# zgchen33/MCGaze

Measured on AMD Instinct MI355X. Metric: clips/sec (7x3x224x224), higher is better.
Workload: dtype f16x3; 1 GPU; full multiclue_gaze_r50 forward (R-50 + FPN + 4 decoder stages + gaze head), 64 clips/GPU x 7 frames x 3x224x224, 64 clips/step; clips_per_gpu=64, clip_length=7, global_clips=64, chunk_frames=0, parallelism=single GPU, trunk_streams=2

## Files before the change

### include/mcgaze_hip.h

```cpp
#ifndef MCGAZE_HIP_H
#define MCGAZE_HIP_H

#include <stddef.h>
#include <stdint.h>

#ifdef __cplusplus
extern "C" {
#endif

#define MCG_ABI_VERSION 18

enum { MCG_OK = 0, MCG_ERR_ARG = 1, MCG_ERR_HIP = 2, MCG_ERR_UNSUPPORTED = 3, MCG_ERR_WORKSPACE = 4 };
typedef enum { MCG_F32 = 0, MCG_BF16 = 1, MCG_F16X3 = 2, MCG_F16 = 3 } mcg_dtype;
#define MCG_ELEM_BYTES(dt) (((dt) == MCG_BF16 || (dt) == MCG_F16) ? 2 : 4)
typedef void* mcg_stream;

int mcg_abi_version(void);
const char* mcg_build_id(void);
const char* mcg_last_error(void);
int mcg_device_info(int* cu_count, size_t* hbm_bytes, char* arch, int arch_len);

int mcg_nchw_to_nhwc(mcg_stream s, mcg_dtype dt, const float* src, void* dst, int N, int C, int H, int W);
int mcg_nhwc_to_nchw(mcg_stream s, mcg_dtype dt, const void* src, float* dst, int N, int C, int H, int W);

enum { MCG_RES_NONE = 0, MCG_RES_ADD = 1, MCG_RES_UPSAMPLE_ADD = 2 };
enum {
  MCG_FLAG_STAGED_GEMM = 1,
  MCG_FLAG_NO_SPECIALISED = 2,
  MCG_FLAG_NO_ATTN_BLOCK = 4
};
typedef struct {
  const void* x;
  const void* w;
  const float* bias;
  const void* residual;
  void* y;
  int N, H, W, Cin, Cout, KH, KW, stride, pad;
  int relu;
  int residual_mode;
  int Hr, Wr;
  const void* x2;
  int Cin2, stride2, H2, W2;
  int tile;
  int flags;
  float wscale;
} mcg_conv_desc;
int mcg_conv2d(mcg_stream s, mcg_dtype dt, const mcg_conv_desc* d);

int mcg_bottleneck_x3(mcg_stream s, const float* x, const float* src2, const void* wstream, const float* bias, float* y, float* z,
                      int frames, int H, int W, int cm, int nsrc, int cn, void* trace);

size_t mcg_conv3x3_wino_x3_weight_bytes(int Cin, int Cout, int g);
int mcg_conv3x3_wino_x3(mcg_stream s, const float* x, const void* u, const float* bias, float* y, int frames, int H, int W,
                        int Cin, int Cout, int relu, int tile, float wscale, int g);

size_t mcg_stem_workspace_bytes(mcg_dtype dt, int N, int H, int W);
int mcg_stem_forward(mcg_stream s, mcg_dtype dt, const float* img, const void* w_stem, const float* bias,
                     void* y, int N, int H, int W, void* ws, size_t ws_bytes, int flags);

int mcg_roi_align(mcg_stream s, mcg_dtype dt, const void* const feats[4], const int feat_h[4], const int feat_w[4],
                  const int strides[4], int C, const float* boxes, int num_boxes, int boxes_per_frame,
                  void* out, int32_t* levels_out);
int mcg_roi_align_indexed(mcg_stream s, mcg_dtype dt, const void* const feats[4], const int feat_h[4], const int feat_w[4],
                          const int strides[4], int C, const float* boxes, int num_boxes, int boxes_per_frame,
                          const int32_t* frame_of, int pyramid_frames, void* out, int32_t* levels_out);

enum {
  MCG_SW_IN_PROJ_W = 0, MCG_SW_IN_PROJ_B, MCG_SW_OUT_PROJ_W, MCG_SW_OUT_PROJ_B, MCG_SW_ATTN_LN_G, MCG_SW_ATTN_LN_B,
  MCG_SW_DYN_W,
  MCG_SW_DYN_B,
  MCG_SW_NORM_IN_G, MCG_SW_NORM_IN_B, MCG_SW_NORM_OUT_G, MCG_SW_NORM_OUT_B,
  MCG_SW_FC_W, MCG_SW_FC_B, MCG_SW_FC_LN_G, MCG_SW_FC_LN_B, MCG_SW_IIC_LN_G, MCG_SW_IIC_LN_B,
  MCG_SW_FFN1_W, MCG_SW_FFN1_B, MCG_SW_FFN2_W, MCG_SW_FFN2_B, MCG_SW_FFN_LN_G, MCG_SW_FFN_LN_B,
  MCG_SW_CLS_FC_W, MCG_SW_CLS_LN_G, MCG_SW_CLS_LN_B,
  MCG_SW_REG_FC_W,
  MCG_SW_REG_LN_G,
  MCG_SW_REG_LN_B,
  MCG_SW_HEAD_CLS_W,
  MCG_SW_HEAD_CLS_B,
  MCG_SW_HEAD_REG_W,
  MCG_SW_HEAD_REG_B,
  MCG_SW_OUT_PROJ_WF, MCG_SW_CLS_FC_WF,
  MCG_SW_REG_FC_WF,
  MCG_SW_IN_PROJ_WF,
  MCG_SW_DYN_WF,
  MCG_SW_COUNT
};
enum {
  MCG_GW_FC_W = 0,
  MCG_GW_LN_G,
  MCG_GW_LN_B,
  MCG_GW_OUT_W,
  MCG_GW_OUT_B,
  MCG_GW_FUSE_W,
  MCG_GW_FUSE_B,
  MCG_GW_COUNT
};

size_t mcg_stage_workspace_bytes(mcg_dtype dt, int num_frames);
int mcg_stage_forward(mcg_stream s, mcg_dtype dt, const void* const weights[MCG_SW_COUNT], const void* roi_feat,
                      const void* obj_in, const float* boxes_in, int num_frames, int clip_length,
                      void* obj_out, float* boxes_out, float* cls_out, const float bbox_stds[4],
                      void* ws, size_t ws_bytes, int flags);
int mcg_stage_forward_ragged(mcg_stream s, mcg_dtype dt, const void* const weights[MCG_SW_COUNT], const void* roi_feat,
                             const void* obj_in, const float* boxes_in, int num_frames, const int* clip_start, int num_clips,
                             int max_clip_length, void* obj_out, float* boxes_out, float* cls_out, const float bbox_stds[4],
                             void* ws, size_t ws_bytes, int flags);

size_t mcg_gaze_head_workspace_bytes(mcg_dtype dt, int num_frames);
int mcg_gaze_head(mcg_stream s, mcg_dtype dt, const void* const weights[MCG_GW_COUNT], const void* obj,
                  int num_frames, float* gaze_out, void* ws, size_t ws_bytes);

typedef struct {
  const void* w;
  const float* bias;
  int cin, cout, k, stride, pad;
  const void* wf;
  float wscale;
  const void* wf4;
} mcg_conv_weights;

typedef struct {
  const void* wstream;
  const float* bias;
  int conv2_index;
  int cm, c, cn;
  int nsrc;
} mcg_fused_block;

typedef struct {
  int blocks[4];
  mcg_conv_weights stem;
  const mcg_conv_weights* convs;
  int num_convs;
  mcg_conv_weights lateral[4];
  mcg_conv_weights fpn_out[4];
  mcg_conv_weights c3_ds[4];
  const float* init_boxes;
  const void* init_feats;
  int num_stages;
  const void* const* stage_weights;
  const void* const* gaze_weights;
  float bbox_stds[4];
  const mcg_fused_block* fused;
  int num_fused;
} mcg_model_weights;

typedef struct mcg_engine mcg_engine;
int mcg_engine_create(mcg_engine** out, const mcg_model_weights* w, mcg_dtype dt);
void mcg_engine_destroy(mcg_engine* e);
int mcg_engine_set_option(mcg_engine* e, const char* name, int value);
int mcg_engine_range_audit(mcg_engine* e, unsigned long long* counts, const char** names, int capacity, int* n_out);
size_t mcg_engine_workspace_bytes(const mcg_engine* e, int num_frames, int H, int W, int chunk_frames);
int mcg_backbone_fpn_forward(mcg_engine* e, mcg_stream s, const float* img, int num_frames, int H, int W,
                             int chunk_frames, void* const pyramid[4], void* ws, size_t ws_bytes);
size_t mcg_trunk_workspace_bytes(const mcg_engine* e, int num_frames, int H, int W, int chunk_frames);
size_t mcg_decoder_workspace_bytes(const mcg_engine* e, int num_frames);
int mcg_decoder_forward(mcg_engine* e, mcg_stream s, const void* const pyramid[4], int num_frames, int clip_length, int H, int W,
                        const int* img_hw, float* gaze_out, float* boxes_out, float* scores_out, void* ws, size_t ws_bytes);
int mcg_decoder_forward_indexed(mcg_engine* e, mcg_stream s, const void* const pyramid[4], int pyramid_frames, const int32_t* frame_of,
                                int num_frames, int clip_length, int H, int W, const int* img_hw, float* gaze_out, float* boxes_out,
                                float* scores_out, void* ws, size_t ws_bytes);
int mcg_decoder_forward_ragged(mcg_engine* e, mcg_stream s, const void* const pyramid[4], int pyramid_frames, const int32_t* frame_of,
                               int num_frames, const int* clip_start, int num_clips, int max_clip_length, int H, int W, const int* img_hw,
                               float* gaze_out, float* boxes_out, float* scores_out, void* ws, size_t ws_bytes);
size_t mcg_deferred_pyramid_bytes(const mcg_engine* e, int num_frames, int H, int W);
int mcg_deferred_pyramid_levels(const mcg_engine* e, void* slot, int num_frames, int H, int W, void* levels[4], int* deferred);
int mcg_backbone_fpn_forward_deferred(mcg_engine* e, mcg_stream s, const float* img, int num_frames, int H, int W, int chunk_frames,
                                      void* slot, size_t slot_bytes, void* ws, size_t ws_bytes);
int mcg_decoder_forward_deferred(mcg_engine* e, mcg_stream s, void* slot, size_t slot_bytes, int num_frames, int clip_length, int H, int W,
                                 const int* img_hw, float* gaze_out, float* boxes_out, float* scores_out, void* ws, size_t ws_bytes);
int mcg_decoder_forward_deferred_ragged(mcg_engine* e, mcg_stream s, void* slot, size_t slot_bytes, int num_frames, const int* clip_start,
                                        int num_clips, int max_clip_length, int H, int W, const int* img_hw, float* gaze_out,
                                        float* boxes_out, float* scores_out, void* ws, size_t ws_bytes);
int mcg_clip_forward(mcg_engine* e, mcg_stream s, const float* img, int num_frames, int clip_length, int H, int W,
                     const int* img_hw, int chunk_frames, float* gaze_out, float* boxes_out, float* scores_out,
                     void* ws, size_t ws_bytes);
int mcg_clip_forward_ragged(mcg_engine* e, mcg_stream s, const float* img, int num_frames, const int* clip_start, int num_clips,
                            int max_clip_length, int H, int W, const int* img_hw, int chunk_frames, float* gaze_out, float* boxes_out,
                            float* scores_out, void* ws, size_t ws_bytes);
int mcg_pyramid_scatter_rows(mcg_stream s, mcg_dtype dt, const void* const src[4], void* const dst[4],
                             int num_frames, int store_rows, int H, int W, const int32_t* row_of);
int mcg_merge_windows(mcg_stream s, const float* gaze, const float* boxes, const float* scores, int num_frames, const float* scale,
                      int scale_per_frame, const int32_t* plan, int num_dst, int max_src, float* store, int store_rows,
                      float person_threshold);
int mcg_smooth_gaze(mcg_stream s, const float* store, int store_rows, const int32_t* plan, int num_out, double alpha, float* out);

typedef struct mcg_frame_desc {
  const void* src;
  int src_h, src_w, src_pitch;
  int crop_y, crop_x, crop_h, crop_w;
  int out_h, out_w;
} mcg_frame_desc;
int mcg_preprocess_frames(mcg_stream stream, const mcg_frame_desc* frames_dev, int num_frames, float* dst, int pad_h, int pad_w,
                          const float mean[3], const float stdinv[3], int to_rgb);
typedef struct mcg_image_desc {
  const void* src;
  int h, w, pitch;
} mcg_image_desc;
int mcg_preprocess_head_crops(mcg_stream s, const mcg_image_desc* images_dev, int num_images, const float* boxes_dev,
                              const int32_t* image_of_dev, int n, double expand, int scale_w, int scale_h, mcg_frame_desc* desc_out_dev,
                              int32_t* img_hw_dev, float* scale_factor_dev, int32_t* flags_dev, float* dst, int pad_h, int pad_w,
                              const float mean[3], const float stdinv[3], int to_rgb);
typedef struct mcg_yuv_coef {
  int y_off, cy, cub, cug, cvg, cvr;
} mcg_yuv_coef;
typedef struct mcg_nv12_image_desc {
  const void* y;
  const void* uv;
  int h, w, pitch_y, pitch_uv;
} mcg_nv12_image_desc;
typedef struct mcg_nv12_frame_desc {
  const void* src;
  int src_h, src_w, src_pitch;
  int crop_y, crop_x, crop_h, crop_w;
  int out_h, out_w;
  const void* uv;
  int uv_pitch;
} mcg_nv12_frame_desc;
int mcg_preprocess_frames_nv12(mcg_stream stream, const mcg_nv12_frame_desc* frames_dev, int num_frames, float* dst, int pad_h, int pad_w,
                               const float mean[3], const float stdinv[3], int to_rgb, const mcg_yuv_coef* coef);
int mcg_preprocess_head_crops_nv12(mcg_stream s, const mcg_nv12_image_desc* images_dev, int num_images, const float* boxes_dev,
                                   const int32_t* image_of_dev, int n, double expand, int scale_w, int scale_h,
                                   mcg_nv12_frame_desc* desc_out_dev, int32_t* img_hw_dev, float* scale_factor_dev, int32_t* flags_dev,
                                   float* dst, int pad_h, int pad_w, const float mean[3], const float stdinv[3], int to_rgb,
                                   const mcg_yuv_coef* coef);

typedef struct mcg_arrow_desc {
  int seg[3][2][2];
  int thickness;
  int x0, y0, x1, y1;
  int image, flag;
  int reserved;
} mcg_arrow_desc;
int mcg_draw_gaze_arrows(mcg_stream s, const mcg_image_desc* images_dev, int num_images, int max_h, int max_w, const float* boxes_dev,
                         const float* gaze_dev, int gaze_stride, const int32_t* image_of_dev, int n, double length, int min_thickness,
                         double thickness_ratio, double tip_length, const unsigned char* color, const unsigned char* colors_dev,
                         mcg_arrow_desc* plan_out_dev, int32_t* flags_dev);
int mcg_draw_gaze_arrows_nv12(mcg_stream s, const mcg_nv12_image_desc* images_dev, int num_images, int max_h, int max_w, const float* boxes_dev,
                              const float* gaze_dev, int gaze_stride, const int32_t* image_of_dev, int n, double length, int min_thickness,
                              double thickness_ratio, double tip_length, const unsigned char* yuv, const unsigned char* yuvs_dev,
                              mcg_arrow_desc* plan_out_dev, int32_t* flags_dev);

size_t mcg_detect_heads_workspace_bytes(int num_images, int num_anchors);
int mcg_detect_heads(mcg_stream s, const float* pred_dev, int num_images, int num_anchors, int num_classes, long long image_stride, int row_stride,
                     int in_h, int in_w, const int32_t* frame_hw_dev , double conf_thres, double iou_thres,
                     int only_class , int agnostic, int max_nms, int max_det,
                     float* boxes_dev , float* scores_dev , int32_t* classes_dev ,
                     int32_t* image_of_dev , int32_t* counts_dev , int32_t* flags_dev ,
                     void* ws_dev, size_t ws_bytes);

enum { MCG_LETTERBOX_U8 = 0, MCG_LETTERBOX_F16 = 1, MCG_LETTERBOX_F32 = 2 };
typedef struct mcg_letterbox_desc {
  mcg_frame_desc frame;
  int top, left;
} mcg_letterbox_desc;
typedef struct mcg_nv12_letterbox_desc {
  mcg_nv12_frame_desc frame;
  int top, left;
} mcg_nv12_letterbox_desc;
int mcg_letterbox_frames(mcg_stream stream, const mcg_letterbox_desc* frames_dev, int num_frames, void* dst, int out_h, int out_w, int out_type,
                         int swap_rb);
int mcg_letterbox_frames_nv12(mcg_stream stream, const mcg_nv12_letterbox_desc* frames_dev, int num_frames, void* dst, int out_h, int out_w,
                              int out_type, int swap_rb, const mcg_yuv_coef* coef);

typedef struct mcg_track_header {
  int32_t next_id;
  int32_t frames_seen;
  int32_t reserved[2];
} mcg_track_header;
typedef struct mcg_track_slot {
  float box[4];
  int32_t id;
  int32_t age;
  int32_t reserved[2];
} mcg_track_slot;
size_t mcg_track_state_bytes(int num_sequences, int slots);
int mcg_track_heads(mcg_stream s, const float* boxes_dev, long long frame_stride, const int32_t* counts_dev, int num_sequences, int num_frames,
                    int max_det, int slots, double match_iou, int max_age, void* state_dev,
                    float* slot_boxes_dev , int32_t* image_of_dev , int32_t* track_id_dev ,
                    int32_t* age_dev , int32_t* det_of_dev , int32_t* flags_dev );

int mcg_live_slots(mcg_stream s, const void* state_dev, int num_cameras, int slots, int tick, int ring_depth, float* crop_boxes_dev,
                   int32_t* image_of_dev, int32_t* ring_id_dev, float* ring_box_dev, int32_t* matched_dev);
int mcg_live_gate(mcg_stream s, const int32_t* ring_id_dev, const float* ring_box_dev, int ring_depth, int num_cameras, int slots, int tick,
                  const int32_t* table_dev, int num_entries, int first_out, int num_out, const float* fused_dev, const float* others_dev,
                  float* fused_smooth_dev, float* others_smooth_dev, int32_t* track_id_dev, int32_t* valid_dev, float* head_box_dev,
                  int32_t* image_of_dev, int32_t* smooth_valid_dev);

int mcg_live_lanes(mcg_stream s, const void* state_dev, int num_cameras, int slots, int lanes, int tick, int ring_depth,
                   int32_t* lane_state_dev, float* crop_boxes_dev, int32_t* image_of_dev, int32_t* ring_id_dev, float* ring_box_dev,
                   int32_t* ring_col_dev, int32_t* lane_of_dev, int32_t* matched_dev, int32_t* overflow_dev);
int mcg_live_gate_lanes(mcg_stream s, const int32_t* ring_id_dev, const float* ring_box_dev, const int32_t* ring_col_dev, int ring_depth,
                        int num_cameras, int slots, int lanes, int tick, const int32_t* table_dev, int num_entries, int first_out, int num_out,
                        const float* fused_dev, const float* others_dev, float* fused_smooth_dev, float* others_smooth_dev,
                        int32_t* track_id_dev, int32_t* valid_dev, int32_t* camera_dev, int32_t* slot_dev, float* head_box_dev,
                        int32_t* image_of_dev, int32_t* smooth_valid_dev);

int mcg_engine_profile_start(mcg_engine* e, int capacity);
int mcg_engine_profile_stop(mcg_engine* e, int* count, float* ms, double* flops, double* algo_bytes, int* cfg, int* shape_mnk, int capacity);
int mcg_bench_backbone_forward(mcg_engine* e, mcg_stream s, const float* img, int num_frames, int H, int W, void* ws, size_t ws_bytes);
int mcg_bench_backbone_levels(const mcg_engine* e, void* ws, int num_frames, int H, int W, void* levels[4]);

#ifdef __cplusplus
}
#endif
#endif
```

### mcgaze_amd/csrc/engine.hip

```cpp
#include "igemm.hpp"
#include "pw_pair.hpp"
#include "pw_single.hpp"
#include "bneck_x3.hpp"
#include "pw_single_x3.hpp"
#include "wino_x3.hpp"

#include <stdarg.h>
#include <stdlib.h>
#include <string.h>

#include <map>
#include <mutex>
#include <string>
#include <vector>

int launch_roi_align(hipStream_t s, mcg_dtype dt, const void* const feats[4], const int feat_h[4], const int feat_w[4],
                     const int strides[4], int C, const float* boxes, int num_boxes, int boxes_per_frame, const int32_t* frame_of,
                     int pyramid_frames, void* out, int32_t* levels_out);
int launch_init_queries(hipStream_t s, mcg_dtype dt, const float* init_boxes, const void* init_feats, const int* img_hw,
                        const int32_t* frame_of, int pyramid_frames, int H, int W, float* boxes, void* obj, int N);
bool roi_mark_supported(int H, int W);
int launch_defer_clear(hipStream_t s, int* p, int n);
int launch_roi_mark(hipStream_t s, const float* boxes, int num_boxes, int boxes_per_frame, int level, int H, int W, int stride, int* state,
                    int* list, int* count);

struct mcg_engine {
  mcg_dtype dt;
  int blocks[4];
  mcg_conv_weights stem;
  std::vector<mcg_conv_weights> convs;
  mcg_conv_weights lateral[4], fpn_out[4], c3_ds[4];
  std::vector<mcg_fused_block> fused;
  bool bneck_fused = true;
  bool bneck_blocked = true;
  int winograd = 1;
  int wino_tile = -1;
  int fpn_deferred = 1;
  static constexpr int kAuditCap = 256;
  unsigned long long* audit_dev = nullptr;
  std::vector<std::string> audit_names;
  const float* init_boxes;
  const void* init_feats;
  int num_stages;
  std::vector<const void*> stage_w;
  const void* gaze_w[MCG_GW_COUNT];
  float stds[4];
  static constexpr int kMaxSplit = 4, kCandidates = 8;
  struct StreamPool* pool = nullptr;
  hipStream_t* cand = nullptr;
  hipEvent_t ev_fork = nullptr, ev_join[kMaxSplit - 1] = {};
  McgCtx ctx;
  Prof prof;
  int trunk_streams = 2;
  int max_range_frames = 0;
  bool pw_single = true;
  bool pw_pair = true;
  std::mutex mu;
};
struct StreamPool {
  hipStream_t cand[mcg_engine::kCandidates] = {};
  hipEvent_t ev_probe[3] = {};
  std::map<hipStream_t, std::vector<int>> side_of;
  std::mutex mu;
  bool ok = false;
};
static StreamPool* stream_pool_for_current_device() {
  static std::mutex g_mu;
  static std::map<int, StreamPool*> g_pools;
  int dev = 0;
  if (hipGetDevice(&dev) != hipSuccess) return nullptr;
  std::lock_guard<std::mutex> lock(g_mu);
  auto it = g_pools.find(dev);
  if (it != g_pools.end()) return it->second;
  StreamPool* p = new StreamPool();
  bool ok = true;
  for (int i = 0; i < mcg_engine::kCandidates; ++i) ok = ok && hipStreamCreateWithFlags(&p->cand[i], hipStreamNonBlocking) == hipSuccess;
  for (int i = 0; i < 3; ++i) ok = ok && hipEventCreate(&p->ev_probe[i]) == hipSuccess;
  p->ok = ok;
  g_pools[dev] = p;
  return p;
}
__global__ void probe_spin_kernel(long long ticks) {
  const long long t0 = wall_clock64();
  while (wall_clock64() - t0 < ticks) {}
}
static const std::vector<int>& side_streams_for(mcg_engine* e, hipStream_t s) {
  StreamPool* p = e->pool;
  std::lock_guard<std::mutex> lock(p->mu);
  auto it = p->side_of.find(s);
  if (it != p->side_of.end()) return it->second;
  std::vector<int> good, rest;
  const long long ticks = 15000;
  for (int c = 0; c < mcg_engine::kCandidates; ++c) {
    bool concurrent = false;
    if (hipEventRecord(p->ev_probe[0], s) == hipSuccess) {
      hipLaunchKernelGGL(probe_spin_kernel, dim3(1), dim3(64), 0, s, ticks);
      hipLaunchKernelGGL(probe_spin_kernel, dim3(1), dim3(64), 0, p->cand[c], ticks);
      float ms = 0.f;
      if (hipEventRecord(p->ev_probe[1], s) == hipSuccess && hipEventRecord(p->ev_probe[2], p->cand[c]) == hipSuccess &&
          hipEventSynchronize(p->ev_probe[1]) == hipSuccess && hipEventSynchronize(p->ev_probe[2]) == hipSuccess &&
          hipEventElapsedTime(&ms, p->ev_probe[0], p->ev_probe[2]) == hipSuccess)
        concurrent = ms < 0.15f * 1.6f;
    }
    (concurrent ? good : rest).push_back(c);
  }
  (void)hipGetLastError();
  good.insert(good.end(), rest.begin(), rest.end());
  return p->side_of.emplace(s, good).first->second;
}
static int range_frame_cap(const mcg_engine* e, int H, int W) {
  const long long per_frame = (long long)(H / 4) * (W / 4) * 256 * (mcg_is16(e->dt) ? 2 : 4);
  long long cap = 0x7FFFFF00ll / (per_frame > 0 ? per_frame : 1);
  if (e->max_range_frames > 0 && e->max_range_frames < cap) cap = e->max_range_frames;
  return cap < 1 ? 1 : (cap > 0x7fffffff ? 0x7fffffff : (int)cap);
}
static const int kMinFramesPerRange = 56;
static int trunk_ranges(const mcg_engine* e, int frames) {
  int k = e->trunk_streams;
  if (k > mcg_engine::kMaxSplit) k = mcg_engine::kMaxSplit;
  while (k > 1 && frames / k < kMinFramesPerRange) --k;
  return k < 1 ? 1 : k;
}

static inline size_t al256(size_t b) { return (b + 255) / 256 * 256; }
static inline size_t esize(mcg_dtype dt) { return mcg_is16(dt) ? 2 : 4; }

extern "C" void mcg_engine_destroy(mcg_engine* e);
extern "C" int mcg_engine_create(mcg_engine** out, const mcg_model_weights* w, mcg_dtype dt) {
  MCG_CHECK_ARG(out && w, "mcg_engine_create: null pointer");
  MCG_CHECK_ARG(dt == MCG_F32 || dt == MCG_BF16 || dt == MCG_F16X3 || dt == MCG_F16, "mcg_engine_create: unknown dtype %d", (int)dt);
  int expect = 0;
  for (int l = 0; l < 4; ++l) {
    MCG_CHECK_ARG(w->blocks[l] > 0, "mcg_engine_create: blocks[%d]=%d", l, w->blocks[l]);
    expect += 3 * w->blocks[l] + 1;
  }
  MCG_CHECK_ARG(w->num_convs == expect && w->convs, "mcg_engine_create: expected %d bottleneck convs, got %d", expect, w->num_convs);
  MCG_CHECK_ARG(w->num_stages > 0 && w->stage_weights && w->gaze_weights && w->init_boxes && w->init_feats, "mcg_engine_create: decoder tables missing");
  for (int i = 0; i < w->num_convs; ++i)
    MCG_CHECK_ARG(w->convs[i].w && w->convs[i].bias, "mcg_engine_create: conv %d has a null pointer", i);
  mcg_engine* e = new mcg_engine();
  e->dt = dt;
  memcpy(e->blocks, w->blocks, sizeof(e->blocks));
  e->stem = w->stem;
  e->convs.assign(w->convs, w->convs + w->num_convs);
  memcpy(e->lateral, w->lateral, sizeof(e->lateral));
  memcpy(e->fpn_out, w->fpn_out, sizeof(e->fpn_out));
  memcpy(e->c3_ds, w->c3_ds, sizeof(e->c3_ds));
  if (w->fused && w->num_fused > 0 && dt == MCG_F16X3) e->fused.assign(w->fused, w->fused + w->num_fused);
  e->init_boxes = w->init_boxes;
  e->init_feats = w->init_feats;
  e->num_stages = w->num_stages;
  e->stage_w.assign(w->stage_weights, w->stage_weights + (size_t)w->num_stages * MCG_SW_COUNT);
  memcpy(e->gaze_w, w->gaze_weights, sizeof(e->gaze_w));
  memcpy(e->stds, w->bbox_stds, sizeof(e->stds));
  bool ok = hipEventCreateWithFlags(&e->ev_fork, hipEventDisableTiming) == hipSuccess;
  e->pool = stream_pool_for_current_device();
  ok = ok && e->pool && e->pool->ok;
  if (e->pool) e->cand = e->pool->cand;
  for (int i = 0; i < mcg_engine::kMaxSplit - 1; ++i) ok = ok && hipEventCreateWithFlags(&e->ev_join[i], hipEventDisableTiming) == hipSuccess;
  if (!ok) {
    mcg_engine_destroy(e);
    mcg_set_error("mcg_engine_create: could not create the side streams / events");
    return MCG_ERR_HIP;
  }
  *out = e;
  return MCG_OK;
}

extern "C" int mcg_engine_set_option(mcg_engine* e, const char* name, int value) {
  MCG_CHECK_ARG(e && name, "mcg_engine_set_option: null pointer");
  std::lock_guard<std::mutex> lock(e->mu);
  if (!strcmp(name, "trunk_streams")) { MCG_CHECK_ARG(value >= 1 && value <= mcg_engine::kMaxSplit, "trunk_streams must be 1..%d", mcg_engine::kMaxSplit); e->trunk_streams = value; }
  else if (!strcmp(name, "max_range_frames")) { MCG_CHECK_ARG(value >= 0, "max_range_frames must be >= 0"); e->max_range_frames = value; }
  else if (!strcmp(name, "tile")) e->ctx.tile = value > 0 ? value : -1;
  else if (!strcmp(name, "staged_gemm")) e->ctx.staged = value != 0;
  else if (!strcmp(name, "conv3x3_c64")) e->ctx.c64 = value != 0;
  else if (!strcmp(name, "stem_fused")) e->ctx.stem_fused = value != 0;
  else if (!strcmp(name, "decoder_chain")) e->ctx.chain = value != 0;
  else if (!strcmp(name, "decoder_attn_block")) e->ctx.attn_block = value != 0;
  else if (!strcmp(name, "pointwise_pair")) e->pw_pair = value != 0;
  else if (!strcmp(name, "pointwise_stream")) e->pw_single = value != 0;
  else if (!strcmp(name, "bottleneck_fused")) e->bneck_fused = value != 0;
  else if (!strcmp(name, "bottleneck_blocked")) e->bneck_blocked = value != 0;
  else if (!strcmp(name, "winograd")) { MCG_CHECK_ARG(value >= 0 && value <= 2, "winograd must be 0, 1 or 2"); e->winograd = value; }
  else if (!strcmp(name, "fpn_deferred")) e->fpn_deferred = value != 0;
  else if (!strcmp(name, "wino_tile")) { MCG_CHECK_ARG(value >= -1 && value <= 3, "wino_tile must be -1 (by grid size) .. 3"); e->wino_tile = value; }
  else if (!strcmp(name, "range_audit")) {
    MCG_CHECK_ARG(!mcg_is16(e->dt) || !value, "range_audit: f32-storage engines only (MCG_F32, MCG_F16X3)");
    if (value && !e->audit_dev) {
      if (hipMalloc((void**)&e->audit_dev, sizeof(unsigned long long) * 2 * mcg_engine::kAuditCap) != hipSuccess) { e->audit_dev = nullptr; mcg_set_error("range_audit: hipMalloc failed"); return MCG_ERR_HIP; }
    }
    if (value && hipMemset(e->audit_dev, 0, sizeof(unsigned long long) * 2 * mcg_engine::kAuditCap) != hipSuccess) { mcg_set_error("range_audit: hipMemset failed"); return MCG_ERR_HIP; }
    if (!value && e->audit_dev) { (void)hipFree(e->audit_dev); e->audit_dev = nullptr; }
    e->audit_names.clear();
  }
  else { mcg_set_error("mcg_engine_set_option: unknown option '%s'", name); return MCG_ERR_ARG; }
  return MCG_OK;
}

extern "C" int mcg_engine_profile_start(mcg_engine* e, int capacity) {
  MCG_CHECK_ARG(e, "mcg_engine_profile_start: null engine");
  std::lock_guard<std::mutex> lock(e->mu);
  if (e->prof.recs) { mcg_set_error("mcg_engine_profile_start: already armed"); return MCG_ERR_ARG; }
  MCG_CHECK_ARG(capacity > 0 && capacity <= (1 << 20), "mcg_engine_profile_start: bad capacity %d", capacity);
  e->prof.recs = new ProfRec[capacity];
  for (int i = 0; i < capacity; ++i) { e->prof.recs[i].a = nullptr; e->prof.recs[i].b = nullptr; }
  for (int i = 0; i < capacity; ++i) {
    if (hipEventCreate(&e->prof.recs[i].a) != hipSuccess || hipEventCreate(&e->prof.recs[i].b) != hipSuccess) {
      for (int j = 0; j <= i; ++j) {
        if (e->prof.recs[j].a) (void)hipEventDestroy(e->prof.recs[j].a);
        if (e->prof.recs[j].b) (void)hipEventDestroy(e->prof.recs[j].b);
      }
      delete[] e->prof.recs;
      e->prof = Prof();
      mcg_set_error("mcg_engine_profile_start: hipEventCreate failed");
      return MCG_ERR_HIP;
    }
  }
  e->prof.cap = capacity; e->prof.n = 0;
  e->ctx.prof = &e->prof;
  return MCG_OK;
}
extern "C" int mcg_engine_profile_stop(mcg_engine* e, int* count, float* ms, double* flops, double* bytes, int* cfg, int* shape, int capacity) {
  MCG_CHECK_ARG(e, "mcg_engine_profile_stop: null engine");
  std::lock_guard<std::mutex> lock(e->mu);
  if (!e->prof.recs) { mcg_set_error("mcg_engine_profile_stop: not armed"); return MCG_ERR_ARG; }
  const int n = e->prof.n;
  int rc = MCG_OK;
  for (int i = 0; i < n; ++i) {
    const ProfRec& r = e->prof.recs[i];
    float t = 0.f;
    if (hipEventSynchronize(r.b) != hipSuccess || hipEventElapsedTime(&t, r.a, r.b) != hipSuccess) rc = MCG_ERR_HIP;
    if (i < capacity) {
      if (ms) ms[i] = t;
      if (flops) flops[i] = r.flops;
      if (bytes) bytes[i] = r.bytes;
      if (cfg) cfg[i] = r.cfg;
      if (shape) { shape[3 * i] = r.shape[0]; shape[3 * i + 1] = r.shape[1]; shape[3 * i + 2] = r.shape[2]; }
    }
  }
  for (int i = 0; i < e->prof.cap; ++i) { (void)hipEventDestroy(e->prof.recs[i].a); (void)hipEventDestroy(e->prof.recs[i].b); }
  delete[] e->prof.recs;
  e->prof = Prof();
  e->ctx.prof = nullptr;
  if (count) *count = n < capacity ? n : capacity;
  if (rc != MCG_OK) mcg_set_error("mcg_engine_profile_stop: event query failed");
  return rc;
}
extern "C" void mcg_engine_destroy(mcg_engine* e) {
  if (!e) return;
  if (e->ev_fork) (void)hipEventDestroy(e->ev_fork);
  for (int i = 0; i < mcg_engine::kMaxSplit - 1; ++i)
    if (e->ev_join[i]) (void)hipEventDestroy(e->ev_join[i]);
  if (e->prof.recs) {
    for (int i = 0; i < e->prof.cap; ++i) { (void)hipEventDestroy(e->prof.recs[i].a); (void)hipEventDestroy(e->prof.recs[i].b); }
    delete[] e->prof.recs;
  }
  if (e->audit_dev) (void)hipFree(e->audit_dev);
  delete e;
}

__global__ void range_audit_kernel(const float* __restrict__ x, long long n, unsigned long long* __restrict__ cnt) {
  unsigned long long big = 0, bad = 0;
  for (long long i = (long long)blockIdx.x * blockDim.x + threadIdx.x; i < n; i += (long long)gridDim.x * blockDim.x) {
    const float v = x[i];
    if (!(fabsf(v) <= 3.4028235e38f)) ++bad;
    else if (fabsf(v) > 65504.f) ++big;
  }
  big = (unsigned long long)wave_sum((float)big) ;
  bad = (unsigned long long)wave_sum((float)bad);
  if ((threadIdx.x & 63) == 0) {
    if (big) atomicAdd(cnt, big);
    if (bad) atomicAdd(cnt + 1, bad);
  }
}
struct AuditCursor { mcg_engine* e; hipStream_t s; int idx; bool naming; };
__attribute__((format(printf, 4, 5))) static void audit_tensor(AuditCursor& a, const void* p, long long elements, const char* fmt, ...) {
  if (!a.e->audit_dev || a.idx >= mcg_engine::kAuditCap) return;
  if (a.naming) {
    char name[64];
    va_list ap;
    va_start(ap, fmt);
    vsnprintf(name, sizeof(name), fmt, ap);
    va_end(ap);
    a.e->audit_names.push_back(name);
  }
  const long long per_thread = 16;
  long long blocks = (elements + 256 * per_thread - 1) / (256 * per_thread);
  if (blocks > 4096) blocks = 4096;
  if (blocks < 1) blocks = 1;
  hipLaunchKernelGGL(range_audit_kernel, dim3((int)blocks), dim3(256), 0, a.s, (const float*)p, elements, a.e->audit_dev + 2 * a.idx);
  ++a.idx;
}

struct TrunkWs {
  char *stem_ws, *x0, *xa, *xb, *o1, *o2, *ds, *c[4], *l[4];
  size_t stem_bytes, big, total;
};
static TrunkWs trunk_layout(mcg_dtype dt, int n, int H, int W, char* base) {
  const size_t es = esize(dt);
  const size_t h2 = H / 4, w2 = W / 4;
  TrunkWs t;
  size_t off = 0;
  auto take = [&](size_t bytes) { char* p = base ? base + off : nullptr; off += al256(bytes); return p; };
  t.stem_bytes = mcg_stem_workspace_bytes(dt, n, H, W);
  t.stem_ws = take(t.stem_bytes);
  t.big = (size_t)n * h2 * w2 * 256 * es;
  t.x0 = take((size_t)n * h2 * w2 * 64 * es);
  t.xa = take(t.big); t.xb = take(t.big);
  t.o1 = take(t.big / 2); t.o2 = take(t.big / 2);
  t.ds = take(t.big);
  for (int i = 0; i < 4; ++i) {
    const size_t hi = (H / 4) >> i, wi = (W / 4) >> i;
    t.c[i] = take((size_t)n * hi * wi * (256u << i) * es);
    t.l[i] = take((size_t)n * hi * wi * 256 * es);
  }
  t.total = off;
  return t;
}

static int wino_kind(const mcg_engine* e, mcg_dtype dt, const mcg_conv_weights& cw, int n, int h, int w, int rm) {
  return (dt == MCG_F16X3 && e->winograd && e->ctx.tile < 0 && cw.k == 3 && cw.stride == 1 && cw.pad == 1 && rm == MCG_RES_NONE)
             ? ((cw.wf4 && e->winograd >= 2 && wino_x3_applicable(n, h, w, cw.cin, cw.cout, 4)) ? 4 : ((cw.wf && wino_x3_applicable(n, h, w, cw.cin, cw.cout, 2)) ? 2 : 0))
             : 0;
}
static WinoParams wino_params(const mcg_conv_weights& cw, int g, const void* x, int n, int h, int w, void* y, int relu) {
  WinoParams wp;
  memset(&wp, 0, sizeof(wp));
  wp.x = (const float*)x; wp.u = g == 4 ? cw.wf4 : cw.wf; wp.bias = cw.bias; wp.y = (float*)y;
  wp.H = h; wp.W = w; wp.frames = n; wp.Cin = cw.cin; wp.Cout = cw.cout; wp.relu = relu; wp.wscale = cw.wscale;
  return wp;
}
static ProfRec* prof_begin_wino(const McgCtx& ctx, hipStream_t s, const mcg_conv_weights& cw, long long M, bool book = true) {
  return prof_begin(ctx, s, 73, (int)M, cw.cout, 9 * cw.cin, book ? 2.0 * M * 9.0 * cw.cin * cw.cout : 0.0,
                    book ? 4.0 * ((double)M * (cw.cin + cw.cout) + 9.0 * cw.cin * cw.cout) : 0.0);
}
static int launch_done(ProfRec* rec, hipStream_t s, int rc, const char* what) {
  prof_end(rec, s);
  if (rc) { mcg_set_error("%s launch failed", what); return MCG_ERR_HIP; }
  return MCG_OK;
}
static mcg_conv_desc conv_desc(mcg_dtype dt, const mcg_conv_weights& cw, const void* x, int n, int h, int w, void* y, int relu,
                               const void* res, int res_mode, int hr, int wr) {
  mcg_conv_desc d;
  memset(&d, 0, sizeof(d));
  d.x = x; d.w = cw.w; d.bias = cw.bias; d.residual = res; d.y = y;
  d.N = n; d.H = h; d.W = w; d.Cin = cw.cin; d.Cout = cw.cout; d.KH = cw.k; d.KW = cw.k; d.stride = cw.stride; d.pad = cw.pad;
  d.relu = relu; d.residual_mode = res_mode; d.Hr = hr; d.Wr = wr;
  d.wscale = dt == MCG_F16X3 ? cw.wscale : 0.f;
  return d;
}
static int conv_call(const mcg_engine* e, hipStream_t s, mcg_dtype dt, const mcg_conv_weights& cw, const void* x, int n, int h, int w, void* y,
                     int relu, const void* res, int res_mode, int hr, int wr) {
  const long long M = (long long)n * h * w;
  const int rm = res ? res_mode : MCG_RES_NONE;
  const long long res_m = rm == MCG_RES_UPSAMPLE_ADD ? (long long)n * hr * wr : M;
  const bool x3 = dt == MCG_F16X3;
  if ((x3 || mcg_is16(dt)) && e->pw_single && e->ctx.tile < 0 && cw.wf && cw.bias && cw.k == 1 && cw.stride == 1 && cw.pad == 0 && M < 0x7fffffffll &&
      (x3 ? pw_single_x3_applicable(cw.cin, cw.cout, rm, M, res_m) : !e->ctx.staged && pw_single_applicable(cw.cin, cw.cout, rm, M, res_m))) {
    PwSingleParams pp;
    memset(&pp, 0, sizeof(pp));
    pp.a = x; pp.res = res; pp.wf = cw.wf; pp.bias = cw.bias; pp.y = y;
    pp.M = (int)M; pp.relu = relu; pp.Ho = h; pp.Wo = w; pp.wscale = x3 ? cw.wscale : 0.f;
    if (rm == MCG_RES_UPSAMPLE_ADD) { pp.Hr = hr; pp.Wr = wr; pp.rscale_h = (float)hr / (float)h; pp.rscale_w = (float)wr / (float)w; }
    ProfRec* rec = prof_begin(e->ctx, s, x3 ? 71 : 61, pp.M, cw.cout, cw.cin, 2.0 * M * cw.cin * cw.cout,
                              (double)esize(dt) * ((double)M * (cw.cin + cw.cout) + (rm == MCG_RES_NONE ? 0.0 : (double)res_m) * cw.cout + (double)cw.cin * cw.cout));
    const int rmode = rm == MCG_RES_NONE ? 0 : (rm == MCG_RES_ADD ? 1 : 2);
    return launch_done(rec, s, x3 ? launch_pw_single_x3(s, pp, cw.cout, rmode) : launch_pw_single(s, pp, cw.cin, cw.cout, rmode, dt),
                       x3 ? "pw_single_x3" : "pw_single");
  }
  const int wg = wino_kind(e, dt, cw, n, h, w, rm);
  if (wg) {
    ProfRec* rec = prof_begin_wino(e->ctx, s, cw, M);
    return launch_done(rec, s, launch_wino_x3(s, wino_params(cw, wg, x, n, h, w, y, relu), e->wino_tile, wg), "wino_x3");
  }
  const mcg_conv_desc d = conv_desc(dt, cw, x, n, h, w, y, relu, res, res_mode, hr, wr);
  return conv2d_ctx(s, dt, &d, e->ctx);
}

struct TrunkCursor {
  const void* x;
  int h, w, ci;
  char *o1, *o2;
  bool o1_ready;
  bool x_blocked;
};
static const mcg_fused_block* fused_tail_at(const mcg_engine* e, int ci, int b) {
  if (!(e->dt == MCG_F16X3 && e->bneck_fused && e->ctx.tile < 0) || ci + 2 >= (int)e->convs.size()) return nullptr;
  const mcg_fused_block* f = nullptr;
  for (const mcg_fused_block& q : e->fused)
    if (q.conv2_index == ci + 1) f = &q;
  if (!f) return nullptr;
  const bool ds = b == 0;
  const mcg_conv_weights &d2 = e->convs[ci + 1], &d3 = e->convs[ci + 2];
  const int kk = ds ? e->convs[ci + 3].cin : 0, ss = ds ? e->convs[ci + 3].stride : 1;
  const int cn_i = ci + (ds ? 4 : 3);
  const bool nx = f->cn == 0 || (cn_i < (int)e->convs.size() && e->convs[cn_i].k == 1 && e->convs[cn_i].stride == 1 && e->convs[cn_i].cout == f->cn && e->convs[cn_i].cin == f->c);
  return (d2.k == 3 && d2.stride == 1 && d2.pad == 1 && d2.cin == f->cm && d2.cout == f->cm && d3.cout == f->c && f->nsrc == (ds ? 2 : 1) && nx &&
          bneck_x3_applicable(f->cm, f->c, f->cn, f->nsrc, kk, ss)) ? f : nullptr;
}
static int fused_tail_step(const mcg_engine* e, hipStream_t s, const TrunkWs& t, AuditCursor& au, TrunkCursor& c, const mcg_fused_block* fb,
                           int n, int l, int b, void* y) {
  const bool has_ds = b == 0;
  const int k2 = has_ds ? e->convs[c.ci + 3].cin : 0;
  BneckParams bp;
  memset(&bp, 0, sizeof(bp));
  bp.x = (const float*)c.o1; bp.res = (const float*)c.x; bp.wstream = (const char*)fb->wstream; bp.bias = fb->bias;
  bp.y = (float*)y; bp.z = (float*)c.o2; bp.H = c.h; bp.W = c.w;
  const long long blk_bytes = (long long)n * ((c.h + bnx::TH - 1) / bnx::TH) * ((c.w + bnx::TW - 1) / bnx::TW) * bnx::NPIX * fb->c * (long long)esize(e->dt);
  const mcg_fused_block* fnext = (b + 1 < e->blocks[l]) ? fused_tail_at(e, c.ci + (has_ds ? 4 : 3), b + 1) : nullptr;
  bp.res_blocked = c.x_blocked ? 1 : 0;
  bp.y_blocked = (e->bneck_blocked && !e->audit_dev && y != (void*)t.c[l] && fb->cn > 0 && fnext && fnext->nsrc == 1 && fnext->c == fb->c &&
                  blk_bytes <= (long long)t.big) ? 1 : 0;
  const double M = (double)n * c.h * c.w;
  ProfRec* rec = prof_begin(e->ctx, s, 70, n * c.h * c.w, fb->c + fb->cn, 9 * fb->cm + fb->cm + k2 + fb->c,
                            2.0 * M * (9.0 * fb->cm * fb->cm + (double)(fb->cm + k2) * fb->c + (double)fb->c * fb->cn),
                            4.0 * (M * (fb->cm + (has_ds ? k2 : fb->c) + fb->c + fb->cn) + 9.0 * fb->cm * fb->cm + (double)(fb->cm + k2) * fb->c + (double)fb->c * fb->cn));
  MCG_TRY(launch_done(rec, s, launch_bneck_x3(s, bp, n, fb->cm, fb->nsrc, fb->cn), "bneck_x3"));
  audit_tensor(au, y, (long long)n * c.h * c.w * fb->c, "layer%d.%d.out (fused tail)", l + 1, b);
  if (fb->cn > 0) {
    audit_tensor(au, c.o2, (long long)n * c.h * c.w * fb->cn, "layer%d.%d.next_conv1 (fused tail)", l + 1, b);
    std::swap(c.o1, c.o2);
    c.o1_ready = true;
  }
  c.x_blocked = bp.y_blocked != 0;
  return MCG_OK;
}
static const mcg_conv_weights* pw_pair_next(const mcg_engine* e, int ci, int l, int b, long long M) {
  const bool has_ds = b == 0;
  const mcg_conv_weights& c3 = e->convs[ci + 2];
  const mcg_conv_weights* c3w = has_ds ? (e->c3_ds[l].w ? &e->c3_ds[l] : nullptr) : &c3;
  const int ci_next = ci + (has_ds ? 4 : 3);
  const mcg_conv_weights* c1n = ci_next < (int)e->convs.size() ? &e->convs[ci_next] : nullptr;
  const int k2 = has_ds ? e->convs[ci + 3].cin : 0;
  return (mcg_is16(e->dt) && e->pw_pair && l == 0 && c3w && c1n && c3w->wf && c1n->wf && c3w->bias && c1n->bias && c1n->k == 1 && c1n->stride == 1 &&
          c1n->cin == c3.cout && pw_pair_applicable(c3.cin, k2, has_ds ? e->convs[ci + 3].stride : 1, c3.cout, c1n->cout, M) && M < 0x7fffffffll)
             ? c1n : nullptr;
}
static int pw_pair_step(const mcg_engine* e, hipStream_t s, TrunkCursor& c, const mcg_conv_weights& c1n, int n, int l, int b, void* y, int ho, int wo) {
  const bool has_ds = b == 0;
  const mcg_conv_weights& c3 = e->convs[c.ci + 2];
  const mcg_conv_weights& c3w = has_ds ? e->c3_ds[l] : c3;
  PwPairParams pp;
  memset(&pp, 0, sizeof(pp));
  pp.a1 = c.o2; pp.K1 = c3.cin;
  if (has_ds) { pp.a2 = c.x; pp.K2 = e->convs[c.ci + 3].cin; pp.stride2 = e->convs[c.ci + 3].stride; pp.H2 = c.h; pp.W2 = c.w; }
  else pp.res = c.x;
  pp.w3f = c3w.wf; pp.b3 = c3w.bias; pp.y = y;
  pp.w1f = c1n.wf; pp.b1 = c1n.bias; pp.z = c.o1;
  pp.M = n * ho * wo; pp.C = c3.cout; pp.C2 = c1n.cout; pp.Ho = ho; pp.Wo = wo;
  ProfRec* rec = prof_begin(e->ctx, s, 60, pp.M, pp.C + pp.C2, pp.K1 + pp.K2, 2.0 * pp.M * ((double)(pp.K1 + pp.K2) * pp.C + (double)pp.C * pp.C2),
                            2.0 * ((double)pp.M * (pp.K1 + pp.K2 + (has_ds ? 0 : pp.C) + pp.C + pp.C2) + (double)(pp.K1 + pp.K2) * pp.C + (double)pp.C * pp.C2));
  MCG_TRY(launch_done(rec, s, launch_pw_pair(s, pp, e->dt), "pw_pair"));
  c.o1_ready = true;
  return MCG_OK;
}
static int conv3_step(const mcg_engine* e, hipStream_t s, const TrunkWs& t, AuditCursor& au, const TrunkCursor& c, int n, int l, int b, void* y,
                      int ho, int wo) {
  const mcg_conv_weights& c3 = e->convs[c.ci + 2];
  if (b == 0 && e->c3_ds[l].w) {
    const mcg_conv_weights& ds = e->convs[c.ci + 3];
    mcg_conv_desc d = conv_desc(e->dt, e->c3_ds[l], c.o2, n, ho, wo, y, 1, nullptr, MCG_RES_NONE, 0, 0);
    d.Cin = c3.cin;
    d.x2 = c.x; d.Cin2 = ds.cin; d.stride2 = ds.stride; d.H2 = c.h; d.W2 = c.w;
    MCG_TRY(conv2d_ctx(s, e->dt, &d, e->ctx));
  } else {
    const void* identity = c.x;
    if (b == 0) {
      MCG_TRY(conv_call(e, s, e->dt, e->convs[c.ci + 3], c.x, n, c.h, c.w, t.ds, 0, nullptr, MCG_RES_NONE, 0, 0));
      identity = t.ds;
    }
    MCG_TRY(conv_call(e, s, e->dt, c3, c.o2, n, ho, wo, y, 1, identity, MCG_RES_ADD, 0, 0));
  }
  audit_tensor(au, y, (long long)n * ho * wo * c3.cout, "layer%d.%d.out", l + 1, b);
  return MCG_OK;
}

static int trunk_chunk(mcg_engine* e, hipStream_t s, const float* img, int f0, int n, int H, int W, void* const pyr[4], char* wsbase,
                       bool backbone_only = false, char* inner0 = nullptr) {
  const mcg_dtype dt = e->dt;
  const size_t es = esize(dt);
  TrunkWs t = trunk_layout(dt, n, H, W, wsbase);
  if (inner0) t.l[0] = inner0 + (size_t)f0 * (H / 4) * (W / 4) * 256 * es;
  MCG_TRY(stem_forward_ctx(s, dt, img + (size_t)f0 * 3 * H * W, e->stem.w, e->stem.bias, t.x0, n, H, W, t.stem_ws, t.stem_bytes, e->ctx));
  AuditCursor au{e, s, 0, e->audit_dev != nullptr && e->audit_names.empty()};
  audit_tensor(au, t.x0, (long long)n * (H / 4) * (W / 4) * 64, "stem");
  TrunkCursor c{t.x0, H / 4, W / 4, 0, t.o1, t.o2, false, false};
  for (int l = 0; l < 4; ++l) {
    for (int b = 0; b < e->blocks[l]; ++b) {
      const mcg_conv_weights &c1 = e->convs[c.ci], &c2 = e->convs[c.ci + 1];
      const int ho = (c.h + 2 * c2.pad - c2.k) / c2.stride + 1, wo = (c.w + 2 * c2.pad - c2.k) / c2.stride + 1;
      void* y = (b == e->blocks[l] - 1) ? (void*)t.c[l] : (c.x == t.xa ? (void*)t.xb : (void*)t.xa);
      if (!c.o1_ready) {
        MCG_TRY(conv_call(e, s, dt, c1, c.x, n, c.h, c.w, c.o1, 1, nullptr, MCG_RES_NONE, 0, 0));
        audit_tensor(au, c.o1, (long long)n * c.h * c.w * c1.cout, "layer%d.%d.conv1", l + 1, b);
      }
      c.o1_ready = false;
      const mcg_fused_block* fb = fused_tail_at(e, c.ci, b);
      if (c.x_blocked && !(fb && fb->nsrc == 1)) { mcg_set_error("trunk: a blocked tensor reached a kernel that does not read that layout"); return MCG_ERR_UNSUPPORTED; }
      if (fb) {
        MCG_TRY(fused_tail_step(e, s, t, au, c, fb, n, l, b, y));
      } else {
        MCG_TRY(conv_call(e, s, dt, c2, c.o1, n, c.h, c.w, c.o2, 1, nullptr, MCG_RES_NONE, 0, 0));
        audit_tensor(au, c.o2, (long long)n * ho * wo * c2.cout, "layer%d.%d.conv2", l + 1, b);
        const mcg_conv_weights* c1n = pw_pair_next(e, c.ci, l, b, (long long)n * ho * wo);
        MCG_TRY(c1n ? pw_pair_step(e, s, c, *c1n, n, l, b, y, ho, wo) : conv3_step(e, s, t, au, c, n, l, b, y, ho, wo));
      }
      c.x = y; c.h = ho; c.w = wo;
      c.ci += b == 0 ? 4 : 3;
    }
  }
  if (backbone_only) return MCG_OK;
  int hs[4], wsz[4];
  for (int i = 0; i < 4; ++i) { hs[i] = (H / 4) >> i; wsz[i] = (W / 4) >> i; }
  for (int i = 3; i >= 0; --i) {
    const void* res = i == 3 ? nullptr : t.l[i + 1];
    MCG_TRY(conv_call(e, s, dt, e->lateral[i], t.c[i], n, hs[i], wsz[i], t.l[i], 0, res, res ? MCG_RES_UPSAMPLE_ADD : MCG_RES_NONE,
                      i == 3 ? 0 : hs[i + 1], i == 3 ? 0 : wsz[i + 1]));
    audit_tensor(au, t.l[i], (long long)n * hs[i] * wsz[i] * 256, "fpn.lateral%d (+ top-down)", i);
  }
  for (int i = inner0 ? 1 : 0; i < 4; ++i) {
    char* dst = (char*)pyr[i] + (size_t)f0 * hs[i] * wsz[i] * 256 * es;
    MCG_TRY(conv_call(e, s, dt, e->fpn_out[i], t.l[i], n, hs[i], wsz[i], dst, 0, nullptr, MCG_RES_NONE, 0, 0));
    audit_tensor(au, dst, (long long)n * hs[i] * wsz[i] * 256, "fpn.P%d", i + 2);
  }
  return MCG_OK;
}

extern "C" int mcg_engine_range_audit(mcg_engine* e, unsigned long long* counts, const char** names, int capacity, int* n_out) {
  MCG_CHECK_ARG(e && counts && n_out && capacity > 0, "mcg_engine_range_audit: bad argument");
  std::lock_guard<std::mutex> lock(e->mu);
  if (!e->audit_dev) { mcg_set_error("mcg_engine_range_audit: the range_audit option is off"); return MCG_ERR_ARG; }
  const int n = (int)e->audit_names.size() < capacity ? (int)e->audit_names.size() : capacity;
  if (hipDeviceSynchronize() != hipSuccess ||
      hipMemcpy(counts, e->audit_dev, sizeof(unsigned long long) * 2 * n, hipMemcpyDeviceToHost) != hipSuccess ||
      hipMemset(e->audit_dev, 0, sizeof(unsigned long long) * 2 * mcg_engine::kAuditCap) != hipSuccess) {
    mcg_set_error("mcg_engine_range_audit: device read failed");
    return MCG_ERR_HIP;
  }
  if (names) for (int i = 0; i < n; ++i) names[i] = e->audit_names[i].c_str();
  *n_out = n;
  return MCG_OK;
}

struct DecWs {
  char *roi, *obj_a, *obj_b, *stage_ws, *gaze_ws;
  float *boxes_a, *boxes_b, *cls;
  size_t stage_bytes, gaze_bytes, total;
};
static DecWs dec_layout(mcg_dtype dt, int N, char* base) {
  const size_t es = esize(dt), R = (size_t)N * 3;
  DecWs c;
  memset(&c, 0, sizeof(c));
  size_t off = 0;
  auto take = [&](size_t bytes) { char* p = base ? base + off : nullptr; off += al256(bytes); return p; };
  c.roi = take(R * 49 * 256 * es);
  c.obj_a = take(R * 256 * es); c.obj_b = take(R * 256 * es);
  c.boxes_a = (float*)take(R * 4 * 4); c.boxes_b = (float*)take(R * 4 * 4); c.cls = (float*)take(R * 4);
  c.stage_bytes = mcg_stage_workspace_bytes(dt, N); c.stage_ws = take(c.stage_bytes);
  c.gaze_bytes = mcg_gaze_head_workspace_bytes(dt, N); c.gaze_ws = take(c.gaze_bytes);
  c.total = off;
  return c;
}
static bool check_shape_ok(int N, int H, int W) { return N > 0 && H >= 32 && W >= 32 && H % 32 == 0 && W % 32 == 0; }
static size_t pyramid_bytes(mcg_dtype dt, int N, int H, int W, int level) {
  return al256((size_t)N * ((H / 4) >> level) * ((W / 4) >> level) * 256 * esize(dt));
}

struct DeferSlot {
  void* p[4];
  char* inner;
  int *state, *count, *list;
  int nblk;
  bool deferred;
  size_t total;
};
static bool fpn_deferred_on(const mcg_engine* e, int N, int H, int W) {
  const mcg_conv_weights& cw = e->fpn_out[0];
  const int h = H / 4, w = W / 4;
  return e->fpn_deferred && e->dt == MCG_F16X3 && !e->audit_dev && e->num_stages > 0 && wino_kind(e, e->dt, cw, N, h, w, MCG_RES_NONE) == 2 &&
         wino_x3_blocks_applicable(N, h, w, cw.cin, cw.cout) && roi_mark_supported(h, w);
}
static DeferSlot defer_layout(const mcg_engine* e, int N, int H, int W, char* base) {
  DeferSlot d;
  memset(&d, 0, sizeof(d));
  size_t off = 0;
  auto take = [&](size_t bytes) { char* p = base ? base + off : nullptr; off += al256(bytes); return p; };
  for (int i = 0; i < 4; ++i) d.p[i] = take(pyramid_bytes(e->dt, N, H, W, i));
  d.deferred = fpn_deferred_on(e, N, H, W);
  if (d.deferred) {
    d.inner = take((size_t)N * (H / 4) * (W / 4) * 256 * esize(e->dt));
    d.nblk = N * wino_x3_blocks_per_frame(H / 4, W / 4);
    d.state = (int*)take(sizeof(int) * ((size_t)d.nblk + e->num_stages));
    d.count = d.state ? d.state + d.nblk : nullptr;
    d.list = (int*)take(sizeof(int) * (size_t)d.nblk * e->num_stages);
  }
  d.total = off;
  return d;
}

extern "C" size_t mcg_trunk_workspace_bytes(const mcg_engine* e, int N, int H, int W, int chunk) {
  if (!e || N <= 0) return 0;
  if (chunk <= 0 || chunk > N) chunk = N;
  if (chunk < N) return trunk_layout(e->dt, chunk, H, W, nullptr).total;
  size_t total = 0;
  const int cap = range_frame_cap(e, H, W);
  for (int k = 1; k <= mcg_engine::kMaxSplit; ++k) {
    const int per = (N + k - 1) / k < cap ? (N + k - 1) / k : cap;
    const size_t t = (size_t)k * al256(trunk_layout(e->dt, per, H, W, nullptr).total);
    if (t > total) total = t;
  }
  return total;
}
extern "C" size_t mcg_decoder_workspace_bytes(const mcg_engine* e, int N) {
  if (!e || N <= 0) return 0;
  return dec_layout(e->dt, N, nullptr).total;
}
extern "C" size_t mcg_engine_workspace_bytes(const mcg_engine* e, int N, int H, int W, int chunk) {
  if (!e || N <= 0) return 0;
  return mcg_trunk_workspace_bytes(e, N, H, W, chunk) + mcg_decoder_workspace_bytes(e, N) + defer_layout(e, N, H, W, nullptr).total;
}
extern "C" size_t mcg_deferred_pyramid_bytes(const mcg_engine* e, int N, int H, int W) {
  if (!e || N <= 0 || check_shape_ok(N, H, W) == false) return 0;
  return defer_layout(e, N, H, W, nullptr).total;
}

static int check_shape(int N, int H, int W) {
  MCG_CHECK_ARG(N > 0, "num_frames must be positive (got %d)", N);
  MCG_CHECK_ARG(H >= 32 && W >= 32 && H % 32 == 0 && W % 32 == 0, "frame size %dx%d must be a multiple of 32 (Pad(size_divisor=32))", H, W);
  return MCG_OK;
}

static int trunk_forward(mcg_engine* e, mcg_stream s_, const float* img, int N, int H, int W, int chunk,
                         void* const pyramid[4], void* ws, size_t ws_bytes, bool backbone_only, char* inner0 = nullptr) {
  MCG_CHECK_ARG(e && img && (pyramid || backbone_only) && ws, "mcg_backbone_fpn_forward: null pointer");
  MCG_TRY(check_shape(N, H, W));
  std::lock_guard<std::mutex> lock(e->mu);
  if (chunk <= 0 || chunk > N) chunk = N;
  const size_t need = mcg_trunk_workspace_bytes(e, N, H, W, chunk);
  if (ws_bytes < need) { mcg_set_error("mcg_backbone_fpn_forward: workspace too small (%zu < %zu)", ws_bytes, need); return MCG_ERR_WORKSPACE; }
  const int k = chunk < N ? 1 : trunk_ranges(e, N), cap = range_frame_cap(e, H, W);
  const int per = chunk < N ? chunk : ((N + k - 1) / k < cap ? (N + k - 1) / k : cap);
  const hipStream_t s = (hipStream_t)s_;
  hipStream_t si[mcg_engine::kMaxSplit] = {s};
  if (k > 1) {
    const std::vector<int>& sides = side_streams_for(e, s);
    for (int i = 1; i < k; ++i) si[i] = e->cand[sides[i - 1]];
    if (hipEventRecord(e->ev_fork, s) != hipSuccess) { mcg_set_error("mcg_backbone_fpn_forward: hipEventRecord failed"); return MCG_ERR_HIP; }
    for (int i = 1; i < k; ++i)
      if (hipStreamWaitEvent(si[i], e->ev_fork, 0) != hipSuccess) { mcg_set_error("mcg_backbone_fpn_forward: hipStreamWaitEvent failed"); return MCG_ERR_HIP; }
  }
  const size_t part_ws = k > 1 ? al256(trunk_layout(e->dt, per, H, W, nullptr).total) : 0;
  int rc = MCG_OK;
  for (int f0 = 0, i = 0; f0 < N && rc == MCG_OK; f0 += per, i = (i + 1) % k)
    rc = trunk_chunk(e, si[i], img, f0, (N - f0) < per ? (N - f0) : per, H, W, pyramid, (char*)ws + (size_t)i * part_ws, backbone_only, inner0);
  for (int i = 1; i < k; ++i) {
    if (hipEventRecord(e->ev_join[i - 1], si[i]) != hipSuccess || hipStreamWaitEvent(s, e->ev_join[i - 1], 0) != hipSuccess) {
      mcg_set_error("mcg_backbone_fpn_forward: join failed");
      rc = rc == MCG_OK ? MCG_ERR_HIP : rc;
    }
  }
  return rc;
}

extern "C" int mcg_bottleneck_x3(mcg_stream s, const float* x, const float* src2, const void* wstream, const float* bias, float* y, float* z,
                                 int frames, int H, int W, int cm, int nsrc, int cn, void* trace) {
  MCG_CHECK_ARG(x && src2 && wstream && bias && y && (z || cn == 0), "mcg_bottleneck_x3: null pointer");
  MCG_CHECK_ARG(frames > 0 && H > 0 && W > 0, "mcg_bottleneck_x3: empty problem");
  MCG_CHECK_ARG(bneck_x3_applicable(cm, 4 * cm, cn, nsrc, 64, 1), "mcg_bottleneck_x3: unsupported shape (cm=%d nsrc=%d cn=%d)", cm, nsrc, cn);
  BneckParams bp;
  memset(&bp, 0, sizeof(bp));
  bp.x = x; bp.res = src2; bp.wstream = (const char*)wstream; bp.bias = bias; bp.y = y; bp.z = z; bp.H = H; bp.W = W; bp.trace = (unsigned long long*)trace;
  if (launch_bneck_x3((hipStream_t)s, bp, frames, cm, nsrc, cn)) { mcg_set_error("mcg_bottleneck_x3: launch failed"); return MCG_ERR_HIP; }
  return MCG_OK;
}

extern "C" size_t mcg_conv3x3_wino_x3_weight_bytes(int Cin, int Cout, int g) {
  return (Cin > 0 && Cout > 0 && Cin % 32 == 0 && Cout % wnx::UNT == 0 && (g == 2 || g == 4)) ? wino_x3_weight_bytes(Cin, Cout, g) : 0;
}
extern "C" int mcg_conv3x3_wino_x3(mcg_stream s, const float* x, const void* u, const float* bias, float* y, int frames, int H, int W,
                                   int Cin, int Cout, int relu, int tile, float wscale, int g) {
  MCG_CHECK_ARG(x && u && y, "mcg_conv3x3_wino_x3: null pointer");
  MCG_CHECK_ARG(tile >= 0 && tile <= 4, "mcg_conv3x3_wino_x3: tile must be 0 (by grid size) .. 4");
  if (!wino_x3_applicable(frames, H, W, Cin, Cout, g)) {
    mcg_set_error("mcg_conv3x3_wino_x3: unsupported shape (frames=%d %dx%d, %d -> %d channels, F(%d,3)): Cin %% 32, Cout %% 128, W <= 62 (F(4,3): W %% 4 == 0, W >= 16), a tile's window within its buffer", frames, H, W, Cin, Cout, g);
    return MCG_ERR_UNSUPPORTED;
  }
  WinoParams wp;
  memset(&wp, 0, sizeof(wp));
  wp.x = x; wp.u = u; wp.bias = bias; wp.y = y; wp.H = H; wp.W = W; wp.frames = frames; wp.Cin = Cin; wp.Cout = Cout; wp.relu = relu;
  wp.wscale = wscale;
  if (launch_wino_x3((hipStream_t)s, wp, tile - 1, g)) { mcg_set_error("mcg_conv3x3_wino_x3: launch failed"); return MCG_ERR_HIP; }
  return MCG_OK;
}

extern "C" int mcg_backbone_fpn_forward(mcg_engine* e, mcg_stream s, const float* img, int N, int H, int W, int chunk,
                                        void* const pyramid[4], void* ws, size_t ws_bytes) {
  return trunk_forward(e, s, img, N, H, W, chunk, pyramid, ws, ws_bytes, false);
}
extern "C" int mcg_bench_backbone_forward(mcg_engine* e, mcg_stream s, const float* img, int N, int H, int W, void* ws, size_t ws_bytes) {
  return trunk_forward(e, s, img, N, H, W, 0, nullptr, ws, ws_bytes, true);
}

extern "C" int mcg_bench_backbone_levels(const mcg_engine* e, void* ws, int N, int H, int W, void* levels[4]) {
  MCG_CHECK_ARG(e && ws && levels, "mcg_bench_backbone_levels: null pointer");
  MCG_TRY(check_shape(N, H, W));
  MCG_CHECK_ARG(trunk_ranges(e, N) == 1 && N <= range_frame_cap(e, H, W), "mcg_bench_backbone_levels: the batch runs as several frame ranges (set trunk_streams = 1)");
  const TrunkWs t = trunk_layout(e->dt, N, H, W, (char*)ws);
  for (int i = 0; i < 4; ++i) levels[i] = t.c[i];
  return MCG_OK;
}

static int defer_stage_forward(const mcg_engine* e, hipStream_t s, const DeferSlot& d, int st, const float* boxes, int N, int h, int w) {
  const mcg_conv_weights& cw = e->fpn_out[0];
  int* list = d.list + (size_t)st * d.nblk;
  MCG_TRY(launch_roi_mark(s, boxes, N * 3, 3, 0, h, w, 4, d.state, list, d.count + st));
  ProfRec* rec = prof_begin_wino(e->ctx, s, cw, (long long)N * h * w, st == 0);
  return launch_done(rec, s, launch_wino_x3_blocks(s, wino_params(cw, 2, d.inner, N, h, w, d.p[0], 0), list, d.count + st, d.nblk), "wino_x3 block");
}

static int decoder_forward(mcg_engine* e, hipStream_t s, const void* const pyramid[4], int pyramid_frames, const int32_t* frame_of, int N,
                           const ClipTable& ct, int H, int W, const int* img_hw, float* gaze_out, float* boxes_out, float* scores_out, void* ws,
                           size_t ws_bytes, const DeferSlot* d = nullptr) {
  MCG_CHECK_ARG(e && pyramid && gaze_out && boxes_out && scores_out && ws, "mcg_decoder_forward: null pointer");
  MCG_TRY(check_shape(N, H, W));
  MCG_TRY(check_clips("mcg_decoder_forward", N, ct));
  DecWs c = dec_layout(e->dt, N, (char*)ws);
  if (ws_bytes < c.total) { mcg_set_error("mcg_decoder_forward: workspace too small (%zu < %zu)", ws_bytes, c.total); return MCG_ERR_WORKSPACE; }
  MCG_TRY(launch_init_queries(s, e->dt, e->init_boxes, e->init_feats, img_hw, frame_of, pyramid_frames, H, W, c.boxes_a, c.obj_a, N));
  int fh[4], fw[4];
  const int strides[4] = {4, 8, 16, 32};
  for (int i = 0; i < 4; ++i) { fh[i] = (H / 4) >> i; fw[i] = (W / 4) >> i; }
  char* obj_in = c.obj_a; char* obj_out = c.obj_b;
  float* b_in = c.boxes_a; float* b_out = c.boxes_b;
  const bool defer = d && d->deferred;
  if (defer) MCG_TRY(launch_defer_clear(s, d->state, d->nblk + e->num_stages));
  for (int st = 0; st < e->num_stages; ++st) {
    if (defer) MCG_TRY(defer_stage_forward(e, s, *d, st, b_in, N, fh[0], fw[0]));
    MCG_TRY(launch_roi_align(s, e->dt, pyramid, fh, fw, strides, 256, b_in, N * 3, 3, frame_of, pyramid_frames, c.roi, nullptr));
    float* bdst = (st == e->num_stages - 1) ? boxes_out : b_out;
    MCG_TRY(stage_forward_ctx(s, e->dt, &e->stage_w[(size_t)st * MCG_SW_COUNT], c.roi, obj_in, b_in, N, ct, obj_out, bdst,
                              c.cls, e->stds, c.stage_ws, c.stage_bytes, e->ctx));
    char* t = obj_in; obj_in = obj_out; obj_out = t;
    if (st != e->num_stages - 1) { float* tb = b_in; b_in = b_out; b_out = tb; }
  }
  MCG_TRY(gaze_head_ctx(s, e->dt, e->gaze_w, obj_in, N, gaze_out, c.gaze_ws, c.gaze_bytes, e->ctx, c.cls, scores_out));
  return MCG_OK;
}

extern "C" int mcg_decoder_forward(mcg_engine* e, mcg_stream s_, const void* const pyramid[4], int N, int clip_length, int H, int W,
                                   const int* img_hw, float* gaze_out, float* boxes_out, float* scores_out, void* ws, size_t ws_bytes) {
  return decoder_forward(e, (hipStream_t)s_, pyramid, N, nullptr, N, ClipTable::uniform(N, clip_length), H, W, img_hw, gaze_out, boxes_out, scores_out, ws,
                         ws_bytes);
}

extern "C" int mcg_decoder_forward_indexed(mcg_engine* e, mcg_stream s_, const void* const pyramid[4], int pyramid_frames, const int32_t* frame_of,
                                           int N, int clip_length, int H, int W, const int* img_hw, float* gaze_out, float* boxes_out,
                                           float* scores_out, void* ws, size_t ws_bytes) {
  MCG_CHECK_ARG(frame_of, "mcg_decoder_forward_indexed: null frame_of (mcg_decoder_forward is the plain path)");
  MCG_CHECK_ARG(pyramid_frames > 0, "mcg_decoder_forward_indexed: empty pyramid store (pyramid_frames=%d)", pyramid_frames);
  return decoder_forward(e, (hipStream_t)s_, pyramid, pyramid_frames, frame_of, N, ClipTable::uniform(N, clip_length), H, W, img_hw, gaze_out, boxes_out,
                         scores_out, ws, ws_bytes);
}

extern "C" int mcg_decoder_forward_ragged(mcg_engine* e, mcg_stream s_, const void* const pyramid[4], int pyramid_frames, const int32_t* frame_of,
                                          int N, const int* clip_start, int num_clips, int max_clip_length, int H, int W, const int* img_hw,
                                          float* gaze_out, float* boxes_out, float* scores_out, void* ws, size_t ws_bytes) {
  MCG_CHECK_ARG(clip_start, "mcg_decoder_forward_ragged: null clip_start (mcg_decoder_forward is the equal-length path)");
  MCG_CHECK_ARG(pyramid_frames > 0, "mcg_decoder_forward_ragged: empty pyramid store (pyramid_frames=%d)", pyramid_frames);
  MCG_CHECK_ARG(frame_of || pyramid_frames == N, "mcg_decoder_forward_ragged: without frame_of the pyramid holds one row per frame (%d rows, %d frames)",
                pyramid_frames, N);
  return decoder_forward(e, (hipStream_t)s_, pyramid, pyramid_frames, frame_of, N, ClipTable{clip_start, num_clips, max_clip_length}, H, W, img_hw,
                         gaze_out, boxes_out, scores_out, ws, ws_bytes);
}

extern "C" int mcg_deferred_pyramid_levels(const mcg_engine* e, void* slot, int N, int H, int W, void* levels[4], int* deferred) {
  MCG_CHECK_ARG(e && slot && levels, "mcg_deferred_pyramid_levels: null pointer");
  MCG_TRY(check_shape(N, H, W));
  const DeferSlot d = defer_layout(e, N, H, W, (char*)slot);
  for (int i = 0; i < 4; ++i) levels[i] = d.p[i];
  if (deferred) *deferred = d.deferred ? 1 : 0;
  return MCG_OK;
}

extern "C" int mcg_backbone_fpn_forward_deferred(mcg_engine* e, mcg_stream s, const float* img, int N, int H, int W, int chunk, void* slot,
                                                 size_t slot_bytes, void* ws, size_t ws_bytes) {
  MCG_CHECK_ARG(e && slot, "mcg_backbone_fpn_forward_deferred: null pointer");
  MCG_TRY(check_shape(N, H, W));
  const DeferSlot d = defer_layout(e, N, H, W, (char*)slot);
  if (slot_bytes < d.total) { mcg_set_error("mcg_backbone_fpn_forward_deferred: slot too small (%zu < %zu)", slot_bytes, d.total); return MCG_ERR_WORKSPACE; }
  return trunk_forward(e, s, img, N, H, W, chunk, d.p, ws, ws_bytes, false, d.deferred ? d.inner : nullptr);
}

static int decoder_forward_deferred(mcg_engine* e, mcg_stream s, void* slot, size_t slot_bytes, int N, const ClipTable& ct, int H, int W,
                                    const int* img_hw, float* gaze_out, float* boxes_out, float* scores_out, void* ws, size_t ws_bytes) {
  MCG_CHECK_ARG(e && slot, "mcg_decoder_forward_deferred: null pointer");
  MCG_TRY(check_shape(N, H, W));
  const DeferSlot d = defer_layout(e, N, H, W, (char*)slot);
  if (slot_bytes < d.total) { mcg_set_error("mcg_decoder_forward_deferred: slot too small (%zu < %zu)", slot_bytes, d.total); return MCG_ERR_WORKSPACE; }
  return decoder_forward(e, (hipStream_t)s, d.p, N, nullptr, N, ct, H, W, img_hw, gaze_out, boxes_out, scores_out, ws, ws_bytes, &d);
}

extern "C" int mcg_decoder_forward_deferred(mcg_engine* e, mcg_stream s, void* slot, size_t slot_bytes, int N, int clip_length, int H, int W,
                                            const int* img_hw, float* gaze_out, float* boxes_out, float* scores_out, void* ws, size_t ws_bytes) {
  return decoder_forward_deferred(e, s, slot, slot_bytes, N, ClipTable::uniform(N, clip_length), H, W, img_hw, gaze_out, boxes_out, scores_out, ws, ws_bytes);
}

extern "C" int mcg_decoder_forward_deferred_ragged(mcg_engine* e, mcg_stream s, void* slot, size_t slot_bytes, int N, const int* clip_start,
                                                   int num_clips, int max_clip_length, int H, int W, const int* img_hw, float* gaze_out,
                                                   float* boxes_out, float* scores_out, void* ws, size_t ws_bytes) {
  MCG_CHECK_ARG(clip_start, "mcg_decoder_forward_deferred_ragged: null clip_start (mcg_decoder_forward_deferred is the equal-length path)");
  return decoder_forward_deferred(e, s, slot, slot_bytes, N, ClipTable{clip_start, num_clips, max_clip_length}, H, W, img_hw, gaze_out, boxes_out,
                                  scores_out, ws, ws_bytes);
}

static int clip_forward(mcg_engine* e, mcg_stream s_, const float* img, int N, const ClipTable& ct, int H, int W, const int* img_hw, int chunk,
                        float* gaze_out, float* boxes_out, float* scores_out, void* ws, size_t ws_bytes) {
  MCG_CHECK_ARG(e && img && gaze_out && boxes_out && scores_out && ws, "mcg_clip_forward: null pointer");
  MCG_TRY(check_shape(N, H, W));
  MCG_TRY(check_clips("mcg_clip_forward", N, ct));
  const size_t need = mcg_engine_workspace_bytes(e, N, H, W, chunk);
  if (ws_bytes < need) { mcg_set_error("mcg_clip_forward: workspace too small (%zu < %zu)", ws_bytes, need); return MCG_ERR_WORKSPACE; }
  char* base = (char*)ws;
  const size_t trunk_bytes = mcg_trunk_workspace_bytes(e, N, H, W, chunk);
  const size_t slot_bytes = defer_layout(e, N, H, W, nullptr).total;
  const size_t off = trunk_bytes + slot_bytes;
  MCG_TRY(mcg_backbone_fpn_forward_deferred(e, s_, img, N, H, W, chunk, base + trunk_bytes, slot_bytes, base, trunk_bytes));
  return decoder_forward_deferred(e, s_, base + trunk_bytes, slot_bytes, N, ct, H, W, img_hw, gaze_out, boxes_out, scores_out, base + off,
                                  ws_bytes - off);
}

extern "C" int mcg_clip_forward(mcg_engine* e, mcg_stream s_, const float* img, int N, int clip_length, int H, int W,
                                const int* img_hw, int chunk, float* gaze_out, float* boxes_out, float* scores_out,
                                void* ws, size_t ws_bytes) {
  return clip_forward(e, s_, img, N, ClipTable::uniform(N, clip_length), H, W, img_hw, chunk, gaze_out, boxes_out, scores_out, ws, ws_bytes);
}

extern "C" int mcg_clip_forward_ragged(mcg_engine* e, mcg_stream s_, const float* img, int N, const int* clip_start, int num_clips,
                                       int max_clip_length, int H, int W, const int* img_hw, int chunk, float* gaze_out, float* boxes_out,
                                       float* scores_out, void* ws, size_t ws_bytes) {
  MCG_CHECK_ARG(clip_start, "mcg_clip_forward_ragged: null clip_start (mcg_clip_forward is the equal-length path)");
  return clip_forward(e, s_, img, N, ClipTable{clip_start, num_clips, max_clip_length}, H, W, img_hw, chunk, gaze_out, boxes_out, scores_out, ws,
                      ws_bytes);
}
```

### mcgaze_amd/csrc/pw_single_x3.hpp

```cpp
#pragma once
#include "pw_single.hpp"

template <int KS, int RES, int NSPLIT>
__global__ __launch_bounds__(256, 2) void pw_single_x3_kernel(const PwSingleParams p) {
  constexpr int PX = 32, K = 16 * KS, N = 128, NF = N * NSPLIT, AROWB = 4 * K, YROWB = 4 * N, GROWB = 4 * NF, ACH = AROWB / 16, YCH = YROWB / 16;
  constexpr int ABYTES = PX * AROWB, YBYTES = PX * YROWB;
  constexpr int NYB = RES ? 2 : 1;
  constexpr int AOFF = NYB * YBYTES;
  constexpr int A_PIECES = ABYTES / 1024 / 4, Y_PIECES = YBYTES / 1024 / 4;
  static_assert(ACH <= 64 && YCH <= 64 && A_PIECES >= 1 && Y_PIECES >= 1 && AOFF + ABYTES <= 80 * 1024, "tile geometry");
  extern __shared__ __attribute__((aligned(16))) char smem[];
  const int tid = threadIdx.x, lane = tid & 63, px = lane & 31, half = lane >> 5;
  const int wave = __builtin_amdgcn_readfirstlane(tid >> 6);
  const int bid = blockIdx.x, nwalkers = gridDim.x / NSPLIT;
  const int nsp = p.many_slices ? bid % NSPLIT : (bid >> 3) % NSPLIT, walker = p.many_slices ? bid / NSPLIT : (bid / (8 * NSPLIT)) * 8 + (bid & 7);
  const float wsc = p.wscale > 0.f ? p.wscale : 1.f;
  float4 breg[4];
#pragma unroll
  for (int q = 0; q < 4; ++q) breg[q] = *(const float4*)(p.bias + nsp * N + wave * 32 + 8 * q + 4 * half);
  auto a_off = [](int r, int chunk) { return r * AROWB + ((chunk ^ (r & (ACH >= 32 ? 31 : 15))) << 4); };
  auto y_off = [](int r, int chunk) { return r * YROWB + ((chunk ^ (r & (YCH >= 32 ? 31 : 15))) << 4); };
  uint4 w[KS][2];
  {
    const char* wb = (const char*)p.wf + ((size_t)(nsp * 4 + wave) * KS * 2 * 64 + lane) * 16;
#pragma unroll
    for (int ks = 0; ks < KS; ++ks) {
      w[ks][0] = *(const uint4*)(wb + (size_t)(2 * ks) * 1024);
      w[ks][1] = *(const uint4*)(wb + (size_t)(2 * ks + 1) * 1024);
    }
  }
  const u32x4 srd_a = make_srd(p.a), srd_r = make_srd(RES ? p.res : p.a);
  const uint32_t lds_base = (uint32_t)(uintptr_t)(__attribute__((address_space(3))) char*)smem;
  constexpr int A_LPR = ACH < 64 ? ACH : 64, Y_LPR = YCH < 64 ? YCH : 64;
  constexpr int A_RPP = 64 / A_LPR, Y_RPP = 64 / Y_LPR;
  const int ntiles = (p.M + PX - 1) / PX;
  auto issue_a = [&](int tile) {
    const int rows_left = p.M - tile * PX;
    const uint32_t so = (uint32_t)tile * ABYTES;
    static_for<A_PIECES>([&](auto jc) {
      constexpr int J = decltype(jc)::value;
      const int row = (wave * A_PIECES + J) * A_RPP + lane / A_LPR, pos = lane % A_LPR;
      const uint32_t vo = row < rows_left ? (uint32_t)(row * AROWB + ((pos ^ (row & (ACH >= 32 ? 31 : 15))) << 4)) : MCG_OOB_OFFSET;
      lds_dma16<AOFF + J * 1024>(vo, srd_a, so, lds_base + wave * (A_PIECES * 1024));
    });
  };
  const int HoWo = p.Ho * p.Wo;
  auto issue_res = [&](int tile, int buf) {
    const int rows_left = p.M - tile * PX;
    static_for<Y_PIECES>([&](auto jc) {
      constexpr int J = decltype(jc)::value;
      const int row = (wave * Y_PIECES + J) * Y_RPP + lane / Y_LPR, pos = lane % Y_LPR;
      const int chunk = pos ^ (row & (YCH >= 32 ? 31 : 15));
      uint32_t vo = MCG_OOB_OFFSET, so = 0;
      if (RES == 1) {
        so = (uint32_t)tile * (PX * GROWB) + nsp * YROWB;
        if (row < rows_left) vo = (uint32_t)(row * GROWB + (chunk << 4));
      } else if (row < rows_left) {
        const int m = tile * PX + row;
        const int f = m / HoWo, rem = m - f * HoWo, ho = rem / p.Wo, wo = rem - ho * p.Wo;
        const int sh = min((int)floorf(ho * p.rscale_h), p.Hr - 1), sw = min((int)floorf(wo * p.rscale_w), p.Wr - 1);
        vo = (uint32_t)((((long long)f * p.Hr + sh) * p.Wr + sw) * GROWB + nsp * YROWB + (chunk << 4));
      }
      lds_dma16<J * 1024>(vo, srd_r, so, lds_base + buf * YBYTES + wave * (Y_PIECES * 1024));
    });
  };
  if (walker < ntiles) {
    if (RES) issue_res(walker, 0);
    issue_a(walker);
  }
  int it = 0;
  for (int tile = walker; tile < ntiles; tile += nwalkers, ++it) {
    const long long m0 = (long long)tile * PX;
    char* s_y = smem + (RES ? (it & 1) * YBYTES : 0);
    const char* s_a = smem + AOFF;
    asm volatile("s_waitcnt vmcnt(0)" ::: "memory");
    __syncthreads();
    const bool more = tile + nwalkers < ntiles;
    if (more && RES) issue_res(tile + nwalkers, (it + 1) & 1);
    f32x16 acc;
#pragma unroll
    for (int r = 0; r < 16; ++r) acc[r] = 0.f;
#pragma unroll
    for (int ks = 0; ks < KS; ++ks) {
      bf16x8 xh, xl;
      split_f32x8(*(const uint4*)(s_a + a_off(px, 4 * ks + 2 * half)), *(const uint4*)(s_a + a_off(px, 4 * ks + 2 * half + 1)), xh, xl);
      acc = x3_mfma(__builtin_bit_cast(bf16x8, w[ks][0]), xl, acc);
      acc = x3_mfma(__builtin_bit_cast(bf16x8, w[ks][1]), xh, acc);
      acc = x3_mfma(__builtin_bit_cast(bf16x8, w[ks][0]), xh, acc);
    }
    __syncthreads();
    if (more) issue_a(tile + nwalkers);
#pragma unroll
    for (int q = 0; q < 4; ++q) {
      const int c0 = wave * 32 + 8 * q + 4 * half;
      char* slot = s_y + y_off(px, c0 >> 2);
      float4 v = make_float4(acc[4 * q] * wsc + breg[q].x, acc[4 * q + 1] * wsc + breg[q].y, acc[4 * q + 2] * wsc + breg[q].z, acc[4 * q + 3] * wsc + breg[q].w);
      if (RES) {
        const float4 rr = *(const float4*)slot;
        v.x += rr.x; v.y += rr.y; v.z += rr.z; v.w += rr.w;
      }
      if (p.relu) { v.x = fmaxf(v.x, 0.f); v.y = fmaxf(v.y, 0.f); v.z = fmaxf(v.z, 0.f); v.w = fmaxf(v.w, 0.f); }
      *(float4*)slot = v;
    }
    __syncthreads();
    for (int idx = tid; idx < PX * YCH; idx += 256) {
      const int r = idx / YCH, c = idx - r * YCH;
      if (m0 + r < p.M) *(uint4*)((float*)p.y + (m0 + r) * NF + nsp * N + c * 4) = *(const uint4*)(s_y + y_off(r, c));
    }
  }
}

static inline bool pw_single_x3_applicable(int K, int N, int res_mode, long long M, long long res_rows) {
  return K == 256 && (N == 256 || N == 1024) && M >= 64 * 1024 && M * 4 * (K > N ? K : N) < MCG_DMA_MAX_BYTES && res_rows * 4 * N < MCG_DMA_MAX_BYTES;
}
template <int KS, int RES, int NSPLIT>
static inline int launch_pw_single_x3_t(hipStream_t s, const PwSingleParams& p) {
  constexpr int kLds = (RES ? 2 : 1) * 32 * 512 + 32 * 64 * KS;
  int cus;
  if (kernel_ready<pw_single_x3_kernel<KS, RES, NSPLIT>>(kLds, &cus)) return 1;
  const int ntiles = (p.M + 31) / 32, unit = 8 * NSPLIT;
  int wgs = 2 * cus / unit * unit;
  const int need = (ntiles + 7) / 8 * unit;
  if (wgs < unit) wgs = unit;
  hipLaunchKernelGGL((pw_single_x3_kernel<KS, RES, NSPLIT>), dim3(need < wgs ? need : wgs), dim3(256), kLds, s, p);
  return hipGetLastError() == hipSuccess ? 0 : 1;
}
static inline int launch_pw_single_x3(hipStream_t s, const PwSingleParams& p, int N, int res_mode) {
  if (N == 256) {
    if (res_mode == 0) return launch_pw_single_x3_t<16, 0, 2>(s, p);
    if (res_mode == 1) return launch_pw_single_x3_t<16, 1, 2>(s, p);
    return launch_pw_single_x3_t<16, 2, 2>(s, p);
  }
  if (res_mode == 0) return launch_pw_single_x3_t<16, 0, 8>(s, p);
  if (res_mode == 1) return launch_pw_single_x3_t<16, 1, 8>(s, p);
  return launch_pw_single_x3_t<16, 2, 8>(s, p);
}

static inline int launch_pw_dyn_x3(hipStream_t s, PwSingleParams p) {
  constexpr int KS = 16, NSPLIT = 256, kLds = 32 * 512 + 32 * 64 * KS;
  int cus;
  if (kernel_ready<pw_single_x3_kernel<KS, 0, NSPLIT>>(kLds, &cus)) return 1;
  const int ntiles = (p.M + 31) / 32;
  int walkers = 2 * cus / NSPLIT;
  if (walkers < 1) walkers = 1;
  if (walkers > ntiles) walkers = ntiles;
  p.many_slices = 1;
  hipLaunchKernelGGL((pw_single_x3_kernel<KS, 0, NSPLIT>), dim3(walkers * NSPLIT), dim3(256), kLds, s, p);
  return hipGetLastError() == hipSuccess ? 0 : 1;
}
```

### mcgaze_amd/csrc/roi_align.hip

```cpp
#include "common.hpp"
#include "roi_sample.hpp"

struct RoiLevels {
  const void* feat[4];
  int h[4], w[4];
  float scale[4];
};

template <typename T>
__global__ __launch_bounds__(256) void roi_align_kernel(RoiLevels lv, int C, const float* __restrict__ boxes, int boxes_per_frame,
                                                        const int32_t* __restrict__ frame_of, int pyramid_frames,
                                                        T* __restrict__ out, int32_t* __restrict__ levels_out, float finest_scale) {
  constexpr int EPC = Elem<T>::kPerChunk;
  constexpr int P = 7, S = 2, NS = P * S;
  __shared__ int s_lo[2][NS], s_hi[2][NS];
  __shared__ float s_l[2][NS], s_h[2][NS];
  __shared__ int s_valid[2][NS];
  const int box = blockIdx.x, tid = threadIdx.x;
  const float x1 = boxes[box * 4 + 0], y1 = boxes[box * 4 + 1], x2 = boxes[box * 4 + 2], y2 = boxes[box * 4 + 3];
  const int level = roi_level(x1, y1, x2, y2, finest_scale);
  const int H = lv.h[level], W = lv.w[level];
  const float ss = lv.scale[level];
  if (tid < 2 * NS) {
    const int axis = tid / NS, i = tid % NS;
    int lo, hi, valid;
    float l;
    roi_axis_sample<P, S>(axis == 0 ? y1 : x1, axis == 0 ? y2 : x2, ss, axis == 0 ? H : W, i, lo, hi, l, valid);
    s_lo[axis][i] = lo; s_hi[axis][i] = hi; s_l[axis][i] = l; s_h[axis][i] = 1.f - l; s_valid[axis][i] = valid;
  }
  if (tid == 0) {
    if (levels_out) levels_out[box] = level;
  }
  __syncthreads();
  int frame = box / boxes_per_frame;
  bool bad_row = false;
  if (frame_of) {
    frame = __builtin_amdgcn_readfirstlane(frame_of[frame]);
    bad_row = frame < 0 || frame >= pyramid_frames;
    if (bad_row) frame = 0;
  }
  const T* __restrict__ F = (const T*)lv.feat[level] + (long long)frame * H * W * C;
  const int groups = C / EPC, bins_per_pass = 256 / groups;
  const int cg = tid % groups, slot = tid / groups;
  if (bad_row) {
    float nan[EPC];
#pragma unroll
    for (int e = 0; e < EPC; ++e) nan[e] = __builtin_nanf("");
    for (int bin = slot; bin < P * P; bin += bins_per_pass)
      *(uint4*)(out + ((long long)box * (P * P) + bin) * C + cg * EPC) = f32_to_chunk(nan, (T*)nullptr);
    return;
  }
  for (int bin = slot; bin < P * P; bin += bins_per_pass) {
    const int ph = bin / P, pw = bin % P;
    float acc[EPC];
#pragma unroll
    for (int e = 0; e < EPC; ++e) acc[e] = 0.f;
#pragma unroll
    for (int iy = 0; iy < S; ++iy) {
      const int yi = ph * S + iy;
#pragma unroll
      for (int ix = 0; ix < S; ++ix) {
        const int xi = pw * S + ix;
        if (!(s_valid[0][yi] && s_valid[1][xi])) continue;
        const int yl = s_lo[0][yi], yh = s_hi[0][yi], xl = s_lo[1][xi], xh = s_hi[1][xi];
        const float ly = s_l[0][yi], hy = s_h[0][yi], lx = s_l[1][xi], hx = s_h[1][xi];
        const float w1 = hy * hx, w2 = hy * lx, w3 = ly * hx, w4 = ly * lx;
        float v1[EPC], v2[EPC], v3[EPC], v4[EPC];
        chunk_to_f32(*(const uint4*)(F + ((long long)yl * W + xl) * C + cg * EPC), v1, (T*)nullptr);
        chunk_to_f32(*(const uint4*)(F + ((long long)yl * W + xh) * C + cg * EPC), v2, (T*)nullptr);
        chunk_to_f32(*(const uint4*)(F + ((long long)yh * W + xl) * C + cg * EPC), v3, (T*)nullptr);
        chunk_to_f32(*(const uint4*)(F + ((long long)yh * W + xh) * C + cg * EPC), v4, (T*)nullptr);
#pragma unroll
        for (int e = 0; e < EPC; ++e) acc[e] += w1 * v1[e] + w2 * v2[e] + w3 * v3[e] + w4 * v4[e];
      }
    }
#pragma unroll
    for (int e = 0; e < EPC; ++e) acc[e] *= (1.0f / (float)(S * S));
    *(uint4*)(out + ((long long)box * (P * P) + bin) * C + cg * EPC) = f32_to_chunk(acc, (T*)nullptr);
  }
}

constexpr int kMarkMaxBlocks = 64;
__global__ __launch_bounds__(256) void roi_mark_kernel(const float* __restrict__ boxes, int boxes_per_frame, int level_deferred, int H, int W,
                                                       float ss, int* __restrict__ state, int* __restrict__ list, int* __restrict__ count,
                                                       float finest_scale) {
  constexpr int P = 7, S = 2, NS = P * S;
  __shared__ int s_hit[2][kMarkMaxBlocks];
  const int box = blockIdx.x, tid = threadIdx.x;
  const float x1 = boxes[box * 4 + 0], y1 = boxes[box * 4 + 1], x2 = boxes[box * 4 + 2], y2 = boxes[box * 4 + 3];
  if (roi_level(x1, y1, x2, y2, finest_scale) != level_deferred) return;
  const int by_n = (H + 7) / 8, bx_n = (W + 7) / 8;
  if (tid < 2 * kMarkMaxBlocks) s_hit[tid / kMarkMaxBlocks][tid % kMarkMaxBlocks] = 0;
  __syncthreads();
  if (tid < 2 * NS) {
    const int axis = tid / NS, i = tid % NS;
    int lo, hi, valid;
    float l;
    roi_axis_sample<P, S>(axis == 0 ? y1 : x1, axis == 0 ? y2 : x2, ss, axis == 0 ? H : W, i, lo, hi, l, valid);
    if (valid) { s_hit[axis][lo >> 3] = 1; s_hit[axis][hi >> 3] = 1; }
  }
  __syncthreads();
  const int frame = box / boxes_per_frame;
  for (int t = tid; t < by_n * bx_n; t += 256) {
    const int by = t / bx_n, bx = t - by * bx_n;
    if (s_hit[0][by] && s_hit[1][bx]) {
      const int id = frame * (by_n * bx_n) + t;
      if (atomicCAS(&state[id], 0, 1) == 0) list[atomicAdd(count, 1)] = id;
    }
  }
}
__global__ void defer_clear_kernel(int* __restrict__ p, int n) {
  for (int i = blockIdx.x * blockDim.x + threadIdx.x; i < n; i += gridDim.x * blockDim.x) p[i] = 0;
}
bool roi_mark_supported(int H, int W) { return (H + 7) / 8 <= kMarkMaxBlocks && (W + 7) / 8 <= kMarkMaxBlocks; }
int launch_defer_clear(hipStream_t s, int* p, int n) {
  const int blocks = (n + 255) / 256 < 1024 ? (n + 255) / 256 : 1024;
  hipLaunchKernelGGL(defer_clear_kernel, dim3(blocks > 0 ? blocks : 1), dim3(256), 0, s, p, n);
  MCG_CHECK_LAUNCH("defer_clear");
  return MCG_OK;
}
int launch_roi_mark(hipStream_t s, const float* boxes, int num_boxes, int boxes_per_frame, int level, int H, int W, int stride, int* state,
                    int* list, int* count) {
  MCG_CHECK_ARG(roi_mark_supported(H, W), "roi_mark: deferred level of %dx%d pixels exceeds %d blocks per axis", H, W, kMarkMaxBlocks);
  hipLaunchKernelGGL(roi_mark_kernel, dim3(num_boxes), dim3(256), 0, s, boxes, boxes_per_frame, level, H, W, 1.0f / (float)stride, state, list,
                     count, 56.f);
  MCG_CHECK_LAUNCH("roi_mark");
  return MCG_OK;
}

int launch_roi_align(hipStream_t s, mcg_dtype dt, const void* const feats[4], const int feat_h[4], const int feat_w[4],
                     const int strides[4], int C, const float* boxes, int num_boxes, int boxes_per_frame, const int32_t* frame_of,
                     int pyramid_frames, void* out, int32_t* levels_out) {
  RoiLevels lv;
  for (int i = 0; i < 4; ++i) {
    lv.feat[i] = feats[i]; lv.h[i] = feat_h[i]; lv.w[i] = feat_w[i];
    lv.scale[i] = 1.0f / (float)strides[i];
  }
  const int epc = mcg_is16(dt) ? 8 : 4;
  MCG_CHECK_ARG(C % epc == 0 && C / epc <= 256 && 256 % (C / epc) == 0, "roi_align: unsupported channel count %d", C);
  dispatch_elem(dt, [&](auto e) {
    hipLaunchKernelGGL(roi_align_kernel<decltype(e)>, dim3(num_boxes), dim3(256), 0, s, lv, C, boxes, boxes_per_frame, frame_of, pyramid_frames, (decltype(e)*)out, levels_out, 56.f);
  });
  MCG_CHECK_LAUNCH("roi_align");
  return MCG_OK;
}

extern "C" int mcg_roi_align(mcg_stream s, mcg_dtype dt, const void* const feats[4], const int feat_h[4], const int feat_w[4],
                             const int strides[4], int C, const float* boxes, int num_boxes, int boxes_per_frame,
                             void* out, int32_t* levels_out) {
  MCG_CHECK_ARG(feats && feat_h && feat_w && strides && boxes && out, "mcg_roi_align: null pointer");
  MCG_CHECK_ARG(num_boxes > 0 && boxes_per_frame > 0, "mcg_roi_align: empty box set");
  for (int i = 0; i < 4; ++i) MCG_CHECK_ARG(feats[i] && feat_h[i] > 0 && feat_w[i] > 0 && strides[i] > 0, "mcg_roi_align: bad level %d", i);
  return launch_roi_align((hipStream_t)s, dt, feats, feat_h, feat_w, strides, C, boxes, num_boxes, boxes_per_frame, nullptr, 0, out, levels_out);
}

extern "C" int mcg_roi_align_indexed(mcg_stream s, mcg_dtype dt, const void* const feats[4], const int feat_h[4], const int feat_w[4],
                                     const int strides[4], int C, const float* boxes, int num_boxes, int boxes_per_frame,
                                     const int32_t* frame_of, int pyramid_frames, void* out, int32_t* levels_out) {
  MCG_CHECK_ARG(feats && feat_h && feat_w && strides && boxes && out && frame_of, "mcg_roi_align_indexed: null pointer");
  MCG_CHECK_ARG(num_boxes > 0 && boxes_per_frame > 0 && pyramid_frames > 0, "mcg_roi_align_indexed: empty box set or pyramid");
  for (int i = 0; i < 4; ++i) MCG_CHECK_ARG(feats[i] && feat_h[i] > 0 && feat_w[i] > 0 && strides[i] > 0, "mcg_roi_align_indexed: bad level %d", i);
  return launch_roi_align((hipStream_t)s, dt, feats, feat_h, feat_w, strides, C, boxes, num_boxes, boxes_per_frame, frame_of, pyramid_frames,
                          out, levels_out);
}
```

### mcgaze_amd/lib.py

```python
import ctypes as C
import os

_HERE = os.path.dirname(os.path.abspath(__file__))
LIB_PATH = os.environ.get('MCGAZE_LIB') or os.path.join(_HERE, 'libmcgaze_hip.so')

MCG_OK = 0
MCG_F32, MCG_BF16, MCG_F16X3, MCG_F16 = 0, 1, 2, 3
ABI_VERSION = 18
RES_NONE, RES_ADD, RES_UPSAMPLE_ADD = 0, 1, 2
FLAG_STAGED_GEMM, FLAG_NO_SPECIALISED, FLAG_NO_ATTN_BLOCK = 1, 2, 4

STAGE_KEYS = [
    'IN_PROJ_W', 'IN_PROJ_B', 'OUT_PROJ_W', 'OUT_PROJ_B', 'ATTN_LN_G', 'ATTN_LN_B', 'DYN_W', 'DYN_B',
    'NORM_IN_G', 'NORM_IN_B', 'NORM_OUT_G', 'NORM_OUT_B', 'FC_W', 'FC_B', 'FC_LN_G', 'FC_LN_B', 'IIC_LN_G', 'IIC_LN_B',
    'FFN1_W', 'FFN1_B', 'FFN2_W', 'FFN2_B', 'FFN_LN_G', 'FFN_LN_B', 'CLS_FC_W', 'CLS_LN_G', 'CLS_LN_B',
    'REG_FC_W', 'REG_LN_G', 'REG_LN_B', 'HEAD_CLS_W', 'HEAD_CLS_B', 'HEAD_REG_W', 'HEAD_REG_B', 'OUT_PROJ_WF', 'CLS_FC_WF', 'REG_FC_WF', 'IN_PROJ_WF', 'DYN_WF']
GAZE_KEYS = ['FC_W', 'LN_G', 'LN_B', 'OUT_W', 'OUT_B', 'FUSE_W', 'FUSE_B']
SW_COUNT, GW_COUNT = len(STAGE_KEYS), len(GAZE_KEYS)

EXPORTS = ['mcg_abi_version', 'mcg_build_id', 'mcg_last_error', 'mcg_device_info', 'mcg_nchw_to_nhwc', 'mcg_nhwc_to_nchw', 'mcg_conv2d',
           'mcg_stem_workspace_bytes', 'mcg_stem_forward', 'mcg_roi_align', 'mcg_stage_workspace_bytes', 'mcg_stage_forward',
           'mcg_gaze_head_workspace_bytes', 'mcg_gaze_head', 'mcg_engine_create', 'mcg_engine_destroy',
           'mcg_engine_workspace_bytes', 'mcg_trunk_workspace_bytes', 'mcg_decoder_workspace_bytes', 'mcg_backbone_fpn_forward',
           'mcg_decoder_forward', 'mcg_clip_forward', 'mcg_preprocess_frames', 'mcg_engine_set_option', 'mcg_engine_profile_start',
           'mcg_engine_profile_stop', 'mcg_bench_backbone_forward', 'mcg_bottleneck_x3', 'mcg_bench_backbone_levels', 'mcg_conv3x3_wino_x3',
           'mcg_conv3x3_wino_x3_weight_bytes', 'mcg_engine_range_audit', 'mcg_roi_align_indexed', 'mcg_decoder_forward_indexed',
           'mcg_deferred_pyramid_bytes', 'mcg_deferred_pyramid_levels', 'mcg_backbone_fpn_forward_deferred', 'mcg_decoder_forward_deferred',
           'mcg_stage_forward_ragged', 'mcg_decoder_forward_ragged', 'mcg_decoder_forward_deferred_ragged', 'mcg_clip_forward_ragged',
           'mcg_pyramid_scatter_rows', 'mcg_preprocess_head_crops', 'mcg_merge_windows', 'mcg_smooth_gaze', 'mcg_preprocess_frames_nv12',
           'mcg_preprocess_head_crops_nv12', 'mcg_draw_gaze_arrows', 'mcg_draw_gaze_arrows_nv12',
           'mcg_detect_heads_workspace_bytes', 'mcg_detect_heads', 'mcg_letterbox_frames', 'mcg_letterbox_frames_nv12',
           'mcg_track_state_bytes', 'mcg_track_heads', 'mcg_live_slots', 'mcg_live_gate', 'mcg_live_lanes', 'mcg_live_gate_lanes']
LETTERBOX_U8, LETTERBOX_F16, LETTERBOX_F32 = 0, 1, 2


class ConvDesc(C.Structure):
    _fields_ = [('x', C.c_void_p), ('w', C.c_void_p), ('bias', C.c_void_p), ('residual', C.c_void_p), ('y', C.c_void_p),
                ('N', C.c_int), ('H', C.c_int), ('W', C.c_int), ('Cin', C.c_int), ('Cout', C.c_int), ('KH', C.c_int),
                ('KW', C.c_int), ('stride', C.c_int), ('pad', C.c_int), ('relu', C.c_int), ('residual_mode', C.c_int),
                ('Hr', C.c_int), ('Wr', C.c_int), ('x2', C.c_void_p), ('Cin2', C.c_int), ('stride2', C.c_int), ('H2', C.c_int),
                ('W2', C.c_int), ('tile', C.c_int), ('flags', C.c_int), ('wscale', C.c_float)]


class ConvWeights(C.Structure):
    _fields_ = [('w', C.c_void_p), ('bias', C.c_void_p), ('cin', C.c_int), ('cout', C.c_int), ('k', C.c_int),
                ('stride', C.c_int), ('pad', C.c_int), ('wf', C.c_void_p), ('wscale', C.c_float), ('wf4', C.c_void_p)]


class FusedBlock(C.Structure):
    _fields_ = [('wstream', C.c_void_p), ('bias', C.c_void_p), ('conv2_index', C.c_int), ('cm', C.c_int), ('c', C.c_int), ('cn', C.c_int),
                ('nsrc', C.c_int)]


class ModelWeights(C.Structure):
    _fields_ = [('blocks', C.c_int * 4), ('stem', ConvWeights), ('convs', C.POINTER(ConvWeights)), ('num_convs', C.c_int),
                ('lateral', ConvWeights * 4), ('fpn_out', ConvWeights * 4), ('c3_ds', ConvWeights * 4), ('init_boxes', C.c_void_p),
                ('init_feats', C.c_void_p), ('num_stages', C.c_int), ('stage_weights', C.POINTER(C.c_void_p)),
                ('gaze_weights', C.POINTER(C.c_void_p)), ('bbox_stds', C.c_float * 4), ('fused', C.POINTER(FusedBlock)), ('num_fused', C.c_int)]


class FrameDesc(C.Structure):
    _fields_ = [('src', C.c_void_p), ('src_h', C.c_int), ('src_w', C.c_int), ('src_pitch', C.c_int), ('crop_y', C.c_int),
                ('crop_x', C.c_int), ('crop_h', C.c_int), ('crop_w', C.c_int), ('out_h', C.c_int), ('out_w', C.c_int)]


class ImageDesc(C.Structure):
    _fields_ = [('src', C.c_void_p), ('h', C.c_int), ('w', C.c_int), ('pitch', C.c_int)]


class YuvCoef(C.Structure):
    _fields_ = [(n, C.c_int) for n in ('y_off', 'cy', 'cub', 'cug', 'cvg', 'cvr')]


class Nv12ImageDesc(C.Structure):
    _fields_ = [('y', C.c_void_p), ('uv', C.c_void_p), ('h', C.c_int), ('w', C.c_int), ('pitch_y', C.c_int), ('pitch_uv', C.c_int)]


class Nv12FrameDesc(C.Structure):
    _fields_ = FrameDesc._fields_ + [('uv', C.c_void_p), ('uv_pitch', C.c_int)]


class LetterboxDesc(C.Structure):
    _fields_ = [('frame', FrameDesc), ('top', C.c_int), ('left', C.c_int)]


class Nv12LetterboxDesc(C.Structure):
    _fields_ = [('frame', Nv12FrameDesc), ('top', C.c_int), ('left', C.c_int)]


class ArrowDesc(C.Structure):
    _fields_ = [('seg', C.c_int * 2 * 2 * 3), ('thickness', C.c_int), ('x0', C.c_int), ('y0', C.c_int), ('x1', C.c_int), ('y1', C.c_int),
                ('image', C.c_int), ('flag', C.c_int), ('reserved', C.c_int)]


class McgError(RuntimeError):
    pass


_lib = None


def load():
    global _lib
    if _lib is not None:
        return _lib
    if not os.path.exists(LIB_PATH):
        raise McgError(f'{LIB_PATH} not found: build it with `python -c "import __graft_entry__ as g; g.build()"` '
                       f'(or `make -C mcgaze_amd/csrc`); mcgaze_amd has no CPU fallback')
    lib = C.CDLL(LIB_PATH)
    vp, i, sz = C.c_void_p, C.c_int, C.c_size_t
    lib.mcg_abi_version.restype = i
    lib.mcg_last_error.restype = C.c_char_p
    lib.mcg_build_id.restype = C.c_char_p
    lib.mcg_device_info.argtypes = [C.POINTER(i), C.POINTER(sz), C.c_char_p, i]
    lib.mcg_nchw_to_nhwc.argtypes = [vp, i, vp, vp, i, i, i, i]
    lib.mcg_nhwc_to_nchw.argtypes = [vp, i, vp, vp, i, i, i, i]
    lib.mcg_conv2d.argtypes = [vp, i, C.POINTER(ConvDesc)]
    lib.mcg_stem_workspace_bytes.restype = sz
    lib.mcg_stem_workspace_bytes.argtypes = [i, i, i, i]
    lib.mcg_stem_forward.argtypes = [vp, i, vp, vp, vp, vp, i, i, i, vp, sz, i]
    lib.mcg_roi_align.argtypes = [vp, i, C.POINTER(vp), C.POINTER(i), C.POINTER(i), C.POINTER(i), i, vp, i, i, vp, vp]
    lib.mcg_roi_align_indexed.argtypes = [vp, i, C.POINTER(vp), C.POINTER(i), C.POINTER(i), C.POINTER(i), i, vp, i, i, vp, i, vp, vp]
    lib.mcg_stage_workspace_bytes.restype = sz
    lib.mcg_stage_workspace_bytes.argtypes = [i, i]
    lib.mcg_stage_forward.argtypes = [vp, i, C.POINTER(vp), vp, vp, vp, i, i, vp, vp, vp, C.POINTER(C.c_float), vp, sz, i]
    lib.mcg_gaze_head_workspace_bytes.restype = sz
    lib.mcg_gaze_head_workspace_bytes.argtypes = [i, i]
    lib.mcg_gaze_head.argtypes = [vp, i, C.POINTER(vp), vp, i, vp, vp, sz]
    lib.mcg_engine_create.argtypes = [C.POINTER(vp), C.POINTER(ModelWeights), i]
    lib.mcg_engine_destroy.argtypes = [vp]
    lib.mcg_engine_destroy.restype = None
    lib.mcg_engine_workspace_bytes.restype = sz
    lib.mcg_engine_workspace_bytes.argtypes = [vp, i, i, i, i]
    lib.mcg_trunk_workspace_bytes.restype = sz
    lib.mcg_trunk_workspace_bytes.argtypes = [vp, i, i, i, i]
    lib.mcg_decoder_workspace_bytes.restype = sz
    lib.mcg_decoder_workspace_bytes.argtypes = [vp, i]
    lib.mcg_decoder_forward.argtypes = [vp, vp, C.POINTER(vp), i, i, i, i, vp, vp, vp, vp, vp, sz]
    lib.mcg_decoder_forward_indexed.argtypes = [vp, vp, C.POINTER(vp), i, vp, i, i, i, i, vp, vp, vp, vp, vp, sz]
    lib.mcg_backbone_fpn_forward.argtypes = [vp, vp, vp, i, i, i, i, C.POINTER(vp), vp, sz]
    lib.mcg_deferred_pyramid_bytes.restype = sz
    lib.mcg_deferred_pyramid_bytes.argtypes = [vp, i, i, i]
    lib.mcg_deferred_pyramid_levels.argtypes = [vp, vp, i, i, i, C.POINTER(vp), C.POINTER(i)]
    lib.mcg_backbone_fpn_forward_deferred.argtypes = [vp, vp, vp, i, i, i, i, vp, sz, vp, sz]
    lib.mcg_decoder_forward_deferred.argtypes = [vp, vp, vp, sz, i, i, i, i, vp, vp, vp, vp, vp, sz]
    lib.mcg_clip_forward.argtypes = [vp, vp, vp, i, i, i, i, vp, i, vp, vp, vp, vp, sz]
    lib.mcg_stage_forward_ragged.argtypes = [vp, i, C.POINTER(vp), vp, vp, vp, i, vp, i, i, vp, vp, vp, C.POINTER(C.c_float), vp, sz, i]
    lib.mcg_decoder_forward_ragged.argtypes = [vp, vp, C.POINTER(vp), i, vp, i, vp, i, i, i, i, vp, vp, vp, vp, vp, sz]
    lib.mcg_decoder_forward_deferred_ragged.argtypes = [vp, vp, vp, sz, i, vp, i, i, i, i, vp, vp, vp, vp, vp, sz]
    lib.mcg_clip_forward_ragged.argtypes = [vp, vp, vp, i, vp, i, i, i, i, vp, i, vp, vp, vp, vp, sz]
    lib.mcg_pyramid_scatter_rows.argtypes = [vp, i, C.POINTER(vp), C.POINTER(vp), i, i, i, i, vp]
    lib.mcg_merge_windows.argtypes = [vp, vp, vp, vp, i, vp, i, vp, i, i, vp, i, C.c_float]
    lib.mcg_smooth_gaze.argtypes = [vp, vp, i, vp, i, C.c_double, vp]
    lib.mcg_preprocess_frames.argtypes =[vp, vp, i, vp, i, i, C.POINTER(C.c_float), C.POINTER(C.c_float), i]
    lib.mcg_preprocess_head_crops.argtypes = [vp, vp, i, vp, vp, i, C.c_double, i, i, vp, vp, vp, vp, vp, i, i, C.POINTER(C.c_float), C.POINTER(C.c_float), i]
    lib.mcg_preprocess_frames_nv12.argtypes = lib.mcg_preprocess_frames.argtypes + [C.POINTER(YuvCoef)]
    lib.mcg_preprocess_head_crops_nv12.argtypes = lib.mcg_preprocess_head_crops.argtypes + [C.POINTER(YuvCoef)]
    u8p = C.POINTER(C.c_ubyte)
    lib.mcg_draw_gaze_arrows.argtypes = [vp, vp, i, i, i, vp, vp, i, vp, i, C.c_double, i, C.c_double, C.c_double, u8p, vp, vp, vp]
    lib.mcg_draw_gaze_arrows_nv12.argtypes = lib.mcg_draw_gaze_arrows.argtypes
    lib.mcg_detect_heads_workspace_bytes.restype = sz
    lib.mcg_detect_heads_workspace_bytes.argtypes = [i, i]
    lib.mcg_detect_heads.argtypes = [vp, vp, i, i, i, C.c_longlong, i, i, i, vp, C.c_double, C.c_double, i, i, i, i, vp, vp, vp, vp, vp, vp, vp, sz]
    lib.mcg_letterbox_frames.argtypes = [vp, vp, i, vp, i, i, i, i]
    lib.mcg_letterbox_frames_nv12.argtypes = lib.mcg_letterbox_frames.argtypes + [C.POINTER(YuvCoef)]
    lib.mcg_track_state_bytes.restype = sz
    lib.mcg_track_state_bytes.argtypes = [i, i]
    lib.mcg_track_heads.argtypes = [vp, vp, C.c_longlong, vp, i, i, i, i, C.c_double, i, vp, vp, vp, vp, vp, vp, vp]
    lib.mcg_live_slots.argtypes = [vp, vp, i, i, i, i, vp, vp, vp, vp, vp]
    lib.mcg_live_gate.argtypes = [vp, vp, vp, i, i, i, i, vp, i, i, i, vp, vp, vp, vp, vp, vp, vp, vp, vp]
    lib.mcg_live_lanes.argtypes = [vp, vp, i, i, i, i, i, vp, vp, vp, vp, vp, vp, vp, vp, vp]
    lib.mcg_live_gate_lanes.argtypes = [vp, vp, vp, vp, i, i, i, i, i, vp, i, i, i, vp, vp, vp, vp, vp, vp, vp, vp, vp, vp, vp]
    lib.mcg_engine_set_option.argtypes = [vp, C.c_char_p, i]
    lib.mcg_engine_profile_start.argtypes = [vp, i]
    lib.mcg_engine_profile_stop.argtypes = [vp, C.POINTER(i), C.POINTER(C.c_float), C.POINTER(C.c_double), C.POINTER(C.c_double), C.POINTER(i), C.POINTER(i), i]
    lib.mcg_bench_backbone_forward.argtypes = [vp, vp, vp, i, i, i, vp, sz]
    lib.mcg_bench_backbone_levels.argtypes = [vp, vp, i, i, i, C.POINTER(vp)]
    lib.mcg_bottleneck_x3.argtypes = [vp, vp, vp, vp, vp, vp, vp, i, i, i, i, i, i, vp]
    lib.mcg_conv3x3_wino_x3.argtypes = [vp, vp, vp, vp, vp, i, i, i, i, i, i, i, C.c_float, i]
    lib.mcg_conv3x3_wino_x3_weight_bytes.restype = sz
    lib.mcg_engine_range_audit.argtypes = [vp, C.POINTER(C.c_ulonglong), C.POINTER(C.c_char_p), i, C.POINTER(i)]
    lib.mcg_conv3x3_wino_x3_weight_bytes.argtypes = [i, i, i]
    for name in EXPORTS:
        fn = getattr(lib, name)
        if fn.restype is C.c_int and name not in ('mcg_abi_version',):
            fn.restype = i
    if lib.mcg_abi_version() != ABI_VERSION:
        raise McgError(f'ABI mismatch: library reports {lib.mcg_abi_version()}, binding expects {ABI_VERSION}')
    _lib = lib
    return lib


def build_id():
    return load().mcg_build_id().decode()


def source_id():
    import hashlib
    src = os.path.join(_HERE, 'csrc')
    names = sorted(n for n in os.listdir(src) if n.endswith('.hip') or n.endswith('.hpp'))
    h = hashlib.sha256()
    for n in names:
        h.update(open(os.path.join(src, n), 'rb').read())
    h.update(open(os.path.join(_HERE, '..', 'include', 'mcgaze_hip.h'), 'rb').read())
    return h.hexdigest()[:16]


def check(rc, what):
    if rc != MCG_OK:
        msg = load().mcg_last_error().decode(errors='replace')
        raise McgError(f'{what} failed (code {rc}): {msg}')
```

Baseline: 3552 clips/s.

## Defer FPN level-0 lateral conv to ROI-touched blocks in the decoder

Extends the deferred FPN path so the level-0 lateral 1x1 conv (with upsample-add from level 1) is no longer computed over the full P2 map in the trunk. Instead, the c2 and l1 tensors are kept in the slot. For each decoder stage, a new kernel marks the 3x3 neighbourhood of the output blocks touched by ROIs, and a listed variant of pw_single_x3 computes the inner map only for those blocks. This removes dense lateral work at the largest pyramid level. In exchange it keeps extra buffers in the slot and adds per-stage marking and sparse-launch overhead, whose cost depends on how many blocks the boxes cover.

```diff
diff --git a/include/mcgaze_hip.h b/include/mcgaze_hip.h
--- a/include/mcgaze_hip.h
+++ b/include/mcgaze_hip.h
@@ -166,6 +166,9 @@
                                float* gaze_out, float* boxes_out, float* scores_out, void* ws, size_t ws_bytes);
 size_t mcg_deferred_pyramid_bytes(const mcg_engine* e, int num_frames, int H, int W);
 int mcg_deferred_pyramid_levels(const mcg_engine* e, void* slot, int num_frames, int H, int W, void* levels[4], int* deferred);
+int mcg_deferred_pyramid_state(const mcg_engine* e, void* slot, int num_frames, int H, int W, void** inner, int** flags, int** counts,
+                               int** lists, int* blocks, int* lateral_deferred);
+int mcg_inner_block_neighbours(int id, int H, int W, int out[9]);
 int mcg_backbone_fpn_forward_deferred(mcg_engine* e, mcg_stream s, const float* img, int num_frames, int H, int W, int chunk_frames,
                                       void* slot, size_t slot_bytes, void* ws, size_t ws_bytes);
 int mcg_decoder_forward_deferred(mcg_engine* e, mcg_stream s, void* slot, size_t slot_bytes, int num_frames, int clip_length, int H, int W,
diff --git a/mcgaze_amd/csrc/engine.hip b/mcgaze_amd/csrc/engine.hip
--- a/mcgaze_amd/csrc/engine.hip
+++ b/mcgaze_amd/csrc/engine.hip
@@ -23,6 +23,7 @@
 int launch_defer_clear(hipStream_t s, int* p, int n);
 int launch_roi_mark(hipStream_t s, const float* boxes, int num_boxes, int boxes_per_frame, int level, int H, int W, int stride, int* state,
                     int* list, int* count);
+int launch_inner_mark(hipStream_t s, const int* out_list, const int* out_count, int H, int W, int nblk, int* state, int* list, int* count);
 
 struct mcg_engine {
   mcg_dtype dt;
@@ -36,6 +37,7 @@
   int winograd = 1;
   int wino_tile = -1;
   int fpn_deferred = 1;
+  int fpn_lateral_deferred = 1;
   static constexpr int kAuditCap = 256;
   unsigned long long* audit_dev = nullptr;
   std::vector<std::string> audit_names;
@@ -184,6 +186,7 @@
   else if (!strcmp(name, "bottleneck_blocked")) e->bneck_blocked = value != 0;
   else if (!strcmp(name, "winograd")) { MCG_CHECK_ARG(value >= 0 && value <= 2, "winograd must be 0, 1 or 2"); e->winograd = value; }
   else if (!strcmp(name, "fpn_deferred")) e->fpn_deferred = value != 0;
+  else if (!strcmp(name, "fpn_lateral_deferred")) e->fpn_lateral_deferred = value != 0;
   else if (!strcmp(name, "wino_tile")) { MCG_CHECK_ARG(value >= -1 && value <= 3, "wino_tile must be -1 (by grid size) .. 3"); e->wino_tile = value; }
   else if (!strcmp(name, "range_audit")) {
     MCG_CHECK_ARG(!mcg_is16(e->dt) || !value, "range_audit: f32-storage engines only (MCG_F32, MCG_F16X3)");
@@ -476,12 +479,19 @@
   return MCG_OK;
 }
 
+struct TrunkKeep { char *inner, *c2, *l1; };
 static int trunk_chunk(mcg_engine* e, hipStream_t s, const float* img, int f0, int n, int H, int W, void* const pyr[4], char* wsbase,
-                       bool backbone_only = false, char* inner0 = nullptr) {
+                       bool backbone_only = false, const TrunkKeep tk = TrunkKeep{nullptr, nullptr, nullptr}) {
   const mcg_dtype dt = e->dt;
   const size_t es = esize(dt);
   TrunkWs t = trunk_layout(dt, n, H, W, wsbase);
+  char* const inner0 = tk.inner;
   if (inner0) t.l[0] = inner0 + (size_t)f0 * (H / 4) * (W / 4) * 256 * es;
+  const bool lateral_deferred = inner0 && tk.c2 && tk.l1;
+  if (lateral_deferred) {
+    t.c[0] = tk.c2 + (size_t)f0 * (H / 4) * (W / 4) * 256 * es;
+    t.l[1] = tk.l1 + (size_t)f0 * (H / 8) * (W / 8) * 256 * es;
+  }
   MCG_TRY(stem_forward_ctx(s, dt, img + (size_t)f0 * 3 * H * W, e->stem.w, e->stem.bias, t.x0, n, H, W, t.stem_ws, t.stem_bytes, e->ctx));
   AuditCursor au{e, s, 0, e->audit_dev != nullptr && e->audit_names.empty()};
   audit_tensor(au, t.x0, (long long)n * (H / 4) * (W / 4) * 64, "stem");
@@ -513,7 +523,7 @@
   if (backbone_only) return MCG_OK;
   int hs[4], wsz[4];
   for (int i = 0; i < 4; ++i) { hs[i] = (H / 4) >> i; wsz[i] = (W / 4) >> i; }
-  for (int i = 3; i >= 0; --i) {
+  for (int i = 3; i >= (lateral_deferred ? 1 : 0); --i) {
     const void* res = i == 3 ? nullptr : t.l[i + 1];
     MCG_TRY(conv_call(e, s, dt, e->lateral[i], t.c[i], n, hs[i], wsz[i], t.l[i], 0, res, res ? MCG_RES_UPSAMPLE_ADD : MCG_RES_NONE,
                       i == 3 ? 0 : hs[i + 1], i == 3 ? 0 : wsz[i + 1]));
@@ -573,6 +583,9 @@
   int *state, *count, *list;
   int nblk;
   bool deferred;
+  bool lateral;
+  char *c2, *l1;
+  int *istate, *icount, *ilist;
   size_t total;
 };
 static bool fpn_deferred_on(const mcg_engine* e, int N, int H, int W) {
@@ -580,6 +593,13 @@
   const int h = H / 4, w = W / 4;
   return e->fpn_deferred && e->dt == MCG_F16X3 && !e->audit_dev && e->num_stages > 0 && wino_kind(e, e->dt, cw, N, h, w, MCG_RES_NONE) == 2 &&
          wino_x3_blocks_applicable(N, h, w, cw.cin, cw.cout) && roi_mark_supported(h, w);
+}
+static bool fpn_lateral_deferred_on(const mcg_engine* e, int N, int H, int W) {
+  const mcg_conv_weights& cw = e->lateral[0];
+  const int h = H / 4, w = W / 4;
+  return e->fpn_lateral_deferred && fpn_deferred_on(e, N, H, W) && e->pw_single && e->ctx.tile < 0 && cw.wf && cw.bias && cw.k == 1 && cw.stride == 1 &&
+         cw.pad == 0 && h % 2 == 0 && w % 2 == 0 &&
+         pw_single_x3_blocks_applicable(cw.cin, cw.cout, h, w, (long long)N * h * w, (long long)N * (h / 2) * (w / 2));
 }
 static DeferSlot defer_layout(const mcg_engine* e, int N, int H, int W, char* base) {
   DeferSlot d;
@@ -591,9 +611,18 @@
   if (d.deferred) {
     d.inner = take((size_t)N * (H / 4) * (W / 4) * 256 * esize(e->dt));
     d.nblk = N * wino_x3_blocks_per_frame(H / 4, W / 4);
-    d.state = (int*)take(sizeof(int) * ((size_t)d.nblk + e->num_stages));
+    d.lateral = fpn_lateral_deferred_on(e, N, H, W);
+    const size_t per = (size_t)d.nblk + e->num_stages;
+    d.state = (int*)take(sizeof(int) * per * (d.lateral ? 2 : 1));
     d.count = d.state ? d.state + d.nblk : nullptr;
     d.list = (int*)take(sizeof(int) * (size_t)d.nblk * e->num_stages);
+    if (d.lateral) {
+      d.istate = d.state ? d.state + per : nullptr;
+      d.icount = d.istate ? d.istate + d.nblk : nullptr;
+      d.ilist = (int*)take(sizeof(int) * (size_t)d.nblk * e->num_stages);
+      d.c2 = take((size_t)N * (H / 4) * (W / 4) * 256 * esize(e->dt));
+      d.l1 = take((size_t)N * (H / 8) * (W / 8) * 256 * esize(e->dt));
+    }
   }
   d.total = off;
   return d;
@@ -632,7 +661,7 @@
 }
 
 static int trunk_forward(mcg_engine* e, mcg_stream s_, const float* img, int N, int H, int W, int chunk,
-                         void* const pyramid[4], void* ws, size_t ws_bytes, bool backbone_only, char* inner0 = nullptr) {
+                         void* const pyramid[4], void* ws, size_t ws_bytes, bool backbone_only, const TrunkKeep tk = TrunkKeep{nullptr, nullptr, nullptr}) {
   MCG_CHECK_ARG(e && img && (pyramid || backbone_only) && ws, "mcg_backbone_fpn_forward: null pointer");
   MCG_TRY(check_shape(N, H, W));
   std::lock_guard<std::mutex> lock(e->mu);
@@ -653,7 +682,7 @@
   const size_t part_ws = k > 1 ? al256(trunk_layout(e->dt, per, H, W, nullptr).total) : 0;
   int rc = MCG_OK;
   for (int f0 = 0, i = 0; f0 < N && rc == MCG_OK; f0 += per, i = (i + 1) % k)
-    rc = trunk_chunk(e, si[i], img, f0, (N - f0) < per ? (N - f0) : per, H, W, pyramid, (char*)ws + (size_t)i * part_ws, backbone_only, inner0);
+    rc = trunk_chunk(e, si[i], img, f0, (N - f0) < per ? (N - f0) : per, H, W, pyramid, (char*)ws + (size_t)i * part_ws, backbone_only, tk);
   for (int i = 1; i < k; ++i) {
     if (hipEventRecord(e->ev_join[i - 1], si[i]) != hipSuccess || hipStreamWaitEvent(s, e->ev_join[i - 1], 0) != hipSuccess) {
       mcg_set_error("mcg_backbone_fpn_forward: join failed");
@@ -715,6 +744,21 @@
   const mcg_conv_weights& cw = e->fpn_out[0];
   int* list = d.list + (size_t)st * d.nblk;
   MCG_TRY(launch_roi_mark(s, boxes, N * 3, 3, 0, h, w, 4, d.state, list, d.count + st));
+  if (d.lateral) {
+    const mcg_conv_weights& lw = e->lateral[0];
+    int* ilist = d.ilist + (size_t)st * d.nblk;
+    MCG_TRY(launch_inner_mark(s, list, d.count + st, h, w, d.nblk, d.istate, ilist, d.icount + st));
+    const long long M = (long long)N * h * w, res_m = (long long)N * (h / 2) * (w / 2);
+    PwSingleParams pp;
+    memset(&pp, 0, sizeof(pp));
+    pp.a = d.c2; pp.res = d.l1; pp.wf = lw.wf; pp.bias = lw.bias; pp.y = d.inner;
+    pp.M = (int)M; pp.relu = 0; pp.Ho = h; pp.Wo = w; pp.wscale = lw.wscale;
+    pp.Hr = h / 2; pp.Wr = w / 2; pp.rscale_h = (float)pp.Hr / (float)h; pp.rscale_w = (float)pp.Wr / (float)w;
+    const bool book = st == 0;
+    ProfRec* lrec = prof_begin(e->ctx, s, 71, pp.M, lw.cout, lw.cin, book ? 2.0 * M * lw.cin * lw.cout : 0.0,
+                               book ? 4.0 * ((double)M * (lw.cin + lw.cout) + (double)res_m * lw.cout + (double)lw.cin * lw.cout) : 0.0);
+    MCG_TRY(launch_done(lrec, s, launch_pw_single_x3_blocks(s, pp, ilist, d.icount + st, d.nblk), "pw_single_x3 block"));
+  }
   ProfRec* rec = prof_begin_wino(e->ctx, s, cw, (long long)N * h * w, st == 0);
   return launch_done(rec, s, launch_wino_x3_blocks(s, wino_params(cw, 2, d.inner, N, h, w, d.p[0], 0), list, d.count + st, d.nblk), "wino_x3 block");
 }
@@ -734,7 +778,7 @@
   char* obj_in = c.obj_a; char* obj_out = c.obj_b;
   float* b_in = c.boxes_a; float* b_out = c.boxes_b;
   const bool defer = d && d->deferred;
-  if (defer) MCG_TRY(launch_defer_clear(s, d->state, d->nblk + e->num_stages));
+  if (defer) MCG_TRY(launch_defer_clear(s, d->state, (d->nblk + e->num_stages) * (d->lateral ? 2 : 1)));
   for (int st = 0; st < e->num_stages; ++st) {
     if (defer) MCG_TRY(defer_stage_forward(e, s, *d, st, b_in, N, fh[0], fw[0]));
     MCG_TRY(launch_roi_align(s, e->dt, pyramid, fh, fw, strides, 256, b_in, N * 3, 3, frame_of, pyramid_frames, c.roi, nullptr));
@@ -789,7 +833,22 @@
   MCG_TRY(check_shape(N, H, W));
   const DeferSlot d = defer_layout(e, N, H, W, (char*)slot);
   if (slot_bytes < d.total) { mcg_set_error("mcg_backbone_fpn_forward_deferred: slot too small (%zu < %zu)", slot_bytes, d.total); return MCG_ERR_WORKSPACE; }
-  return trunk_forward(e, s, img, N, H, W, chunk, d.p, ws, ws_bytes, false, d.deferred ? d.inner : nullptr);
+  return trunk_forward(e, s, img, N, H, W, chunk, d.p, ws, ws_bytes, false,
+                       TrunkKeep{d.deferred ? d.inner : nullptr, d.lateral ? d.c2 : nullptr, d.lateral ? d.l1 : nullptr});
+}
+
+extern "C" int mcg_deferred_pyramid_state(const mcg_engine* e, void* slot, int N, int H, int W, void** inner, int** flags, int** counts, int** lists,
+                                          int* blocks, int* lateral_deferred) {
+  MCG_CHECK_ARG(e && slot, "mcg_deferred_pyramid_state: null pointer");
+  MCG_TRY(check_shape(N, H, W));
+  const DeferSlot d = defer_layout(e, N, H, W, (char*)slot);
+  if (inner) *inner = d.inner;
+  if (flags) *flags = d.istate;
+  if (counts) *counts = d.icount;
+  if (lists) *lists = d.ilist;
+  if (blocks) *blocks = d.nblk;
+  if (lateral_deferred) *lateral_deferred = d.lateral ? 1 : 0;
+  return MCG_OK;
 }
 
 static int decoder_forward_deferred(mcg_engine* e, mcg_stream s, void* slot, size_t slot_bytes, int N, const ClipTable& ct, int H, int W,
diff --git a/mcgaze_amd/csrc/pw_single_x3.hpp b/mcgaze_amd/csrc/pw_single_x3.hpp
--- a/mcgaze_amd/csrc/pw_single_x3.hpp
+++ b/mcgaze_amd/csrc/pw_single_x3.hpp
@@ -1,8 +1,14 @@
 #pragma once
 #include "pw_single.hpp"
 
-template <int KS, int RES, int NSPLIT>
-__global__ __launch_bounds__(256, 2) void pw_single_x3_kernel(const PwSingleParams p) {
+struct PwBlockList {
+  const int* list;
+  const int* count;
+  int bxn, bpf, nblk;
+};
+
+template <int KS, int RES, int NSPLIT, bool LISTED>
+__device__ __forceinline__ void pw_single_x3_body(const PwSingleParams& p, const PwBlockList& bl) {
   constexpr int PX = 32, K = 16 * KS, N = 128, NF = N * NSPLIT, AROWB = 4 * K, YROWB = 4 * N, GROWB = 4 * NF, ACH = AROWB / 16, YCH = YROWB / 16;
   constexpr int ABYTES = PX * AROWB, YBYTES = PX * YROWB;
   constexpr int NYB = RES ? 2 : 1;
@@ -14,6 +20,11 @@
   const int wave = __builtin_amdgcn_readfirstlane(tid >> 6);
   const int bid = blockIdx.x, nwalkers = gridDim.x / NSPLIT;
   const int nsp = p.many_slices ? bid % NSPLIT : (bid >> 3) % NSPLIT, walker = p.many_slices ? bid / NSPLIT : (bid / (8 * NSPLIT)) * 8 + (bid & 7);
+  int listed_tiles = 0;
+  if constexpr (LISTED) {
+    listed_tiles = 2 * __builtin_amdgcn_readfirstlane(*bl.count);
+    if (walker >= listed_tiles) return;
+  }
   const float wsc = p.wscale > 0.f ? p.wscale : 1.f;
   float4 breg[4];
 #pragma unroll
@@ -33,20 +44,28 @@
   const uint32_t lds_base = (uint32_t)(uintptr_t)(__attribute__((address_space(3))) char*)smem;
   constexpr int A_LPR = ACH < 64 ? ACH : 64, Y_LPR = YCH < 64 ? YCH : 64;
   constexpr int A_RPP = 64 / A_LPR, Y_RPP = 64 / Y_LPR;
-  const int ntiles = (p.M + PX - 1) / PX;
-  auto issue_a = [&](int tile) {
-    const int rows_left = p.M - tile * PX;
-    const uint32_t so = (uint32_t)tile * ABYTES;
+  const int ntiles = LISTED ? listed_tiles : (p.M + PX - 1) / PX;
+  auto tile_origin = [&](int tile) {
+    const int blk = __builtin_amdgcn_readfirstlane(bl.list[tile >> 1]);
+    if (blk < 0 || blk >= bl.nblk) return -1;
+    const int f = blk / bl.bpf, rem = blk - f * bl.bpf, by = rem / bl.bxn, bx = rem - by * bl.bxn;
+    return (f * p.Ho + by * 8 + (tile & 1) * 4) * p.Wo + bx * 8;
+  };
+  auto listed_pixel = [&](int org, int r) { return org + (r >> 3) * p.Wo + (r & 7); };
+  auto issue_a = [&](int tile, int org) {
+    const int rows_left = LISTED ? (org >= 0 ? PX : 0) : p.M - tile * PX;
+    const uint32_t so = LISTED ? 0u : (uint32_t)tile * ABYTES;
     static_for<A_PIECES>([&](auto jc) {
       constexpr int J = decltype(jc)::value;
       const int row = (wave * A_PIECES + J) * A_RPP + lane / A_LPR, pos = lane % A_LPR;
-      const uint32_t vo = row < rows_left ? (uint32_t)(row * AROWB + ((pos ^ (row & (ACH >= 32 ? 31 : 15))) << 4)) : MCG_OOB_OFFSET;
+      const uint32_t grow = LISTED ? (uint32_t)listed_pixel(org, row) : (uint32_t)row;
+      const uint32_t vo = row < rows_left ? grow * AROWB + (uint32_t)((pos ^ (row & (ACH >= 32 ? 31 : 15))) << 4) : MCG_OOB_OFFSET;
       lds_dma16<AOFF + J * 1024>(vo, srd_a, so, lds_base + wave * (A_PIECES * 1024));
     });
   };
   const int HoWo = p.Ho * p.Wo;
-  auto issue_res = [&](int tile, int buf) {
-    const int rows_left = p.M - tile * PX;
+  auto issue_res = [&](int tile, int buf, int org) {
+    const int rows_left = LISTED ? (org >= 0 ? PX : 0) : p.M - tile * PX;
     static_for<Y_PIECES>([&](auto jc) {
       constexpr int J = decltype(jc)::value;
       const int row = (wave * Y_PIECES + J) * Y_RPP + lane / Y_LPR, pos = lane % Y_LPR;
@@ -56,7 +75,7 @@
         so = (uint32_t)tile * (PX * GROWB) + nsp * YROWB;
         if (row < rows_left) vo = (uint32_t)(row * GROWB + (chunk << 4));
       } else if (row < rows_left) {
-        const int m = tile * PX + row;
+        const int m = LISTED ? listed_pixel(org, row) : tile * PX + row;
         const int f = m / HoWo, rem = m - f * HoWo, ho = rem / p.Wo, wo = rem - ho * p.Wo;
         const int sh = min((int)floorf(ho * p.rscale_h), p.Hr - 1), sw = min((int)floorf(wo * p.rscale_w), p.Wr - 1);
         vo = (uint32_t)((((long long)f * p.Hr + sh) * p.Wr + sw) * GROWB + nsp * YROWB + (chunk << 4));
@@ -64,9 +83,11 @@
       lds_dma16<J * 1024>(vo, srd_r, so, lds_base + buf * YBYTES + wave * (Y_PIECES * 1024));
     });
   };
+  int org = 0, org_next = 0;
   if (walker < ntiles) {
-    if (RES) issue_res(walker, 0);
-    issue_a(walker);
+    if constexpr (LISTED) org = tile_origin(walker);
+    if (RES) issue_res(walker, 0, org);
+    issue_a(walker, org);
   }
   int it = 0;
   for (int tile = walker; tile < ntiles; tile += nwalkers, ++it) {
@@ -76,7 +97,8 @@
     asm volatile("s_waitcnt vmcnt(0)" ::: "memory");
     __syncthreads();
     const bool more = tile + nwalkers < ntiles;
-    if (more && RES) issue_res(tile + nwalkers, (it + 1) & 1);
+    if constexpr (LISTED) { if (more) org_next = tile_origin(tile + nwalkers); }
+    if (more && RES) issue_res(tile + nwalkers, (it + 1) & 1, org_next);
     f32x16 acc;
 #pragma unroll
     for (int r = 0; r < 16; ++r) acc[r] = 0.f;
@@ -89,7 +111,7 @@
       acc = x3_mfma(__builtin_bit_cast(bf16x8, w[ks][0]), xh, acc);
     }
     __syncthreads();
-    if (more) issue_a(tile + nwalkers);
+    if (more) issue_a(tile + nwalkers, org_next);
 #pragma unroll
     for (int q = 0; q < 4; ++q) {
       const int c0 = wave * 32 + 8 * q + 4 * half;
@@ -105,9 +127,22 @@
     __syncthreads();
     for (int idx = tid; idx < PX * YCH; idx += 256) {
       const int r = idx / YCH, c = idx - r * YCH;
-      if (m0 + r < p.M) *(uint4*)((float*)p.y + (m0 + r) * NF + nsp * N + c * 4) = *(const uint4*)(s_y + y_off(r, c));
-    }
-  }
+      if constexpr (LISTED) {
+        if (org >= 0) *(uint4*)((float*)p.y + (long long)listed_pixel(org, r) * NF + nsp * N + c * 4) = *(const uint4*)(s_y + y_off(r, c));
+      } else {
+        if (m0 + r < p.M) *(uint4*)((float*)p.y + (m0 + r) * NF + nsp * N + c * 4) = *(const uint4*)(s_y + y_off(r, c));
+      }
+    }
+    if constexpr (LISTED) org = org_next;
+  }
+}
+template <int KS, int RES, int NSPLIT>
+__global__ __launch_bounds__(256, 2) void pw_single_x3_kernel(const PwSingleParams p) {
+  pw_single_x3_body<KS, RES, NSPLIT, false>(p, PwBlockList{});
+}
+template <int KS, int NSPLIT>
+__global__ __launch_bounds__(256, 2) void pw_single_x3_blocks_kernel(const PwSingleParams p, const PwBlockList bl) {
+  pw_single_x3_body<KS, 2, NSPLIT, true>(p, bl);
 }
 
 static inline bool pw_single_x3_applicable(int K, int N, int res_mode, long long M, long long res_rows) {
@@ -136,6 +171,23 @@
   return launch_pw_single_x3_t<16, 2, 8>(s, p);
 }
 
+static inline bool pw_single_x3_blocks_applicable(int K, int N, int Ho, int Wo, long long M, long long res_rows) {
+  return K == 256 && N == 256 && Ho > 0 && Wo > 0 && Ho % 8 == 0 && Wo % 8 == 0 && M * 4 * K < MCG_DMA_MAX_BYTES && res_rows * 4 * N < MCG_DMA_MAX_BYTES;
+}
+static inline int launch_pw_single_x3_blocks(hipStream_t s, const PwSingleParams& p, const int* list, const int* count, int max_blocks) {
+  constexpr int KS = 16, NSPLIT = 2, kLds = 2 * 32 * 512 + 32 * 64 * KS;
+  int cus;
+  if (kernel_ready<pw_single_x3_blocks_kernel<KS, NSPLIT>>(kLds, &cus)) return 1;
+  PwBlockList bl;
+  bl.list = list; bl.count = count; bl.bxn = p.Wo / 8; bl.bpf = (p.Ho / 8) * (p.Wo / 8); bl.nblk = max_blocks;
+  const int unit = 8 * NSPLIT;
+  int wgs = 2 * cus / unit * unit;
+  const int need = (2 * max_blocks + 7) / 8 * unit;
+  if (wgs < unit) wgs = unit;
+  hipLaunchKernelGGL((pw_single_x3_blocks_kernel<KS, NSPLIT>), dim3(need < wgs ? need : wgs), dim3(256), kLds, s, p, bl);
+  return hipGetLastError() == hipSuccess ? 0 : 1;
+}
+
 static inline int launch_pw_dyn_x3(hipStream_t s, PwSingleParams p) {
   constexpr int KS = 16, NSPLIT = 256, kLds = 32 * 512 + 32 * 64 * KS;
   int cus;
diff --git a/mcgaze_amd/csrc/roi_align.hip b/mcgaze_amd/csrc/roi_align.hip
--- a/mcgaze_amd/csrc/roi_align.hip
+++ b/mcgaze_amd/csrc/roi_align.hip
@@ -109,6 +109,36 @@
     }
   }
 }
+__host__ __device__ inline int inner_neighbour(int id, int k, int by_n, int bx_n) {
+  const int bpf = by_n * bx_n, f = id / bpf, rem = id - f * bpf, by = rem / bx_n + k / 3 - 1, bx = rem % bx_n + k % 3 - 1;
+  return (by < 0 || by >= by_n || bx < 0 || bx >= bx_n) ? -1 : f * bpf + by * bx_n + bx;
+}
+__global__ __launch_bounds__(256) void inner_mark_kernel(const int* __restrict__ out_list, const int* __restrict__ out_count, int by_n, int bx_n,
+                                                         int nblk, int* __restrict__ state, int* __restrict__ list, int* __restrict__ count) {
+  const int n = min(*out_count, nblk) * 9;
+  for (int t = blockIdx.x * blockDim.x + threadIdx.x; t < n; t += gridDim.x * blockDim.x) {
+    const int src = out_list[t / 9];
+    if (src < 0 || src >= nblk) continue;
+    const int id = inner_neighbour(src, t % 9, by_n, bx_n);
+    if (id >= 0 && atomicCAS(&state[id], 0, 1) == 0) list[atomicAdd(count, 1)] = id;
+  }
+}
+int launch_inner_mark(hipStream_t s, const int* out_list, const int* out_count, int H, int W, int nblk, int* state, int* list, int* count) {
+  const long long threads = (long long)nblk * 9;
+  const int blocks = (int)((threads + 255) / 256 < 1024 ? (threads + 255) / 256 : 1024);
+  hipLaunchKernelGGL(inner_mark_kernel, dim3(blocks > 0 ? blocks : 1), dim3(256), 0, s, out_list, out_count, (H + 7) / 8, (W + 7) / 8, nblk, state,
+                     list, count);
+  MCG_CHECK_LAUNCH("inner_mark");
+  return MCG_OK;
+}
+extern "C" int mcg_inner_block_neighbours(int id, int H, int W, int out[9]) {
+  int n = 0;
+  for (int k = 0; k < 9; ++k) {
+    const int v = inner_neighbour(id, k, (H + 7) / 8, (W + 7) / 8);
+    if (v >= 0) out[n++] = v;
+  }
+  return n;
+}
 __global__ void defer_clear_kernel(int* __restrict__ p, int n) {
   for (int i = blockIdx.x * blockDim.x + threadIdx.x; i < n; i += gridDim.x * blockDim.x) p[i] = 0;
 }
diff --git a/mcgaze_amd/lib.py b/mcgaze_amd/lib.py
--- a/mcgaze_amd/lib.py
+++ b/mcgaze_amd/lib.py
@@ -30,7 +30,8 @@
            'mcg_pyramid_scatter_rows', 'mcg_preprocess_head_crops', 'mcg_merge_windows', 'mcg_smooth_gaze', 'mcg_preprocess_frames_nv12',
            'mcg_preprocess_head_crops_nv12', 'mcg_draw_gaze_arrows', 'mcg_draw_gaze_arrows_nv12',
            'mcg_detect_heads_workspace_bytes', 'mcg_detect_heads', 'mcg_letterbox_frames', 'mcg_letterbox_frames_nv12',
-           'mcg_track_state_bytes', 'mcg_track_heads', 'mcg_live_slots', 'mcg_live_gate', 'mcg_live_lanes', 'mcg_live_gate_lanes']
+           'mcg_track_state_bytes', 'mcg_track_heads', 'mcg_live_slots', 'mcg_live_gate', 'mcg_live_lanes', 'mcg_live_gate_lanes',
+           'mcg_deferred_pyramid_state', 'mcg_inner_block_neighbours']
 LETTERBOX_U8, LETTERBOX_F16, LETTERBOX_F32 = 0, 1, 2
 
 
@@ -142,6 +143,8 @@
     lib.mcg_deferred_pyramid_bytes.restype = sz
     lib.mcg_deferred_pyramid_bytes.argtypes = [vp, i, i, i]
     lib.mcg_deferred_pyramid_levels.argtypes = [vp, vp, i, i, i, C.POINTER(vp), C.POINTER(i)]
+    lib.mcg_deferred_pyramid_state.argtypes = [vp, vp, i, i, i, C.POINTER(vp), C.POINTER(vp), C.POINTER(vp), C.POINTER(vp), C.POINTER(i), C.POINTER(i)]
+    lib.mcg_inner_block_neighbours.argtypes = [i, i, i, C.POINTER(i)]
     lib.mcg_backbone_fpn_forward_deferred.argtypes = [vp, vp, vp, i, i, i, i, vp, sz, vp, sz]
     lib.mcg_decoder_forward_deferred.argtypes = [vp, vp, vp, sz, i, i, i, i, vp, vp, vp, vp, vp, sz]
     lib.mcg_clip_forward.argtypes = [vp, vp, vp, i, i, i, i, vp, i, vp, vp, vp, vp, sz]
```

Result: faster. 3588 clips/s, median of 6 (+1.0%).
